# maksimt/rri_nmf

Hardware: AMD Instinct MI355X
Metric: RRI sweeps/sec and achieved HBM GB/s on dense X (n x d, rank k) (higher is better)
Workload: dtype f64

## Files before the change

### include/rri_hip.h

```cpp
#ifndef RRI_HIP_H
#define RRI_HIP_H

#include <stdint.h>
#include <stddef.h>

#ifdef __cplusplus
extern "C" {
#endif

#define RRI_ABI_VERSION 1
#define RRI_GRAM_SLICES 8
#define RRI_MAX_K 1024
#define RRI_MAX_TOPN 64
#define RRI_MAX_COOC_WORDS 32

typedef struct rri_ctx rri_ctx;
typedef struct rri_comm rri_comm;
#define RRI_COMM_ID_BYTES 128

typedef int32_t rri_status;
enum {
    RRI_OK = 0,
    RRI_PAUSED = 1,
    RRI_ERR_INVALID = -1,
// ... 83 lines not shown
rri_status rri_rank_entries(rri_ctx* ctx, const int64_t* rows, int64_t count,
                            const int64_t* tgt_indptr, const int32_t* tgt_indices,
                            const int64_t* excl_indptr, const int32_t* excl_indices,
                            double clip_lo, double clip_hi,
                            int32_t* rank_out, double* val_out, int32_t* eligible_out);
rri_status rri_cooccurrence_counts(rri_ctx* ctx, const int64_t* indptr, const int32_t* indices,
                                   int64_t n_rows, int64_t n_cols,
                                   const int32_t* words, int32_t n_groups, int32_t group_size,
                                   int64_t* df_out, int64_t* codf_out);
rri_status rri_entries_loglik(rri_ctx* ctx, const int64_t* rows, int64_t count,
                              const int64_t* indptr, const int32_t* indices, const double* values,
                              double floor, double* ll_out, double* mass_out, int64_t* floored_out);
enum { RRI_I32 = 8, RRI_I64 = 9 };
#define RRI_CORPUS_INFO_FIELDS 10
typedef struct rri_corpus rri_corpus;
rri_status rri_corpus_create(rri_ctx* ctx, rri_corpus** out, int64_t n_rows, int64_t n_cols, int64_t nnz_stored,
                             const void* indptr, int32_t indptr_dtype, const void* indices, int32_t indices_dtype,
                             const void* values, int32_t values_dtype, int32_t on_device);
rri_status rri_corpus_destroy(rri_corpus* corpus);
rri_status rri_corpus_info(const rri_corpus* corpus, int64_t* out, int32_t n, double* ingest_ms);
rri_status rri_corpus_get(rri_ctx* ctx, const rri_corpus* corpus, int64_t* indptr_out, int32_t* indices_out, double* values_out);
rri_status rri_corpus_memory(int64_t* corpora, int64_t* bytes);
rri_status rri_corpus_cooccurrence_counts(rri_ctx* ctx, const rri_corpus* corpus, const int32_t* words, int32_t n_groups,
                                          int32_t group_size, int64_t* df_out, int64_t* codf_out);
rri_status rri_corpus_entries_loglik(rri_ctx* ctx, const rri_corpus* corpus, const int64_t* rows, double floor,
                                     double* ll_out, double* mass_out, int64_t* floored_out);
#define RRI_SPARSE_STORE_INFO_FIELDS 10
rri_status rri_upload_X_corpus(rri_ctx* ctx, const rri_corpus* corpus);
rri_status rri_sparse_store_get(rri_ctx* ctx, int32_t which, int64_t* info, int32_t n_info, int64_t* segptr, uint16_t* idx,
                                int32_t* perm, void* val, int32_t* work);
rri_status rri_snapshot(rri_ctx* ctx);
rri_status rri_rollback(rri_ctx* ctx);

rri_status rri_X_times(rri_ctx* ctx, const double* B, int32_t m, double* out);
rri_status rri_Xt_times(rri_ctx* ctx, const double* Q, int32_t m, double* out);
rri_status rri_range_finder(rri_ctx* ctx, const double* Q0, int32_t m, int32_t n_iter, int32_t transpose, double* Q_out,
                            double* B_out);
rri_status rri_sparse_range_finder(rri_ctx* ctx, const double* Q0, int32_t m, int32_t n_iter, int32_t transpose, double* Q_out,
                                   double* B_out);

rri_status rri_column_positive_counts(rri_ctx* ctx, double* df_out);
rri_status rri_scale_X(rri_ctx* ctx, const double* col_scale, int32_t normalize_rows);
rri_status rri_set_X_scales(rri_ctx* ctx, const double* row_scale, const double* col_scale);
rri_status rri_get_X_scales(rri_ctx* ctx, double* row_out, double* col_out);
rri_status rri_csr_column_positive_counts(rri_ctx* ctx, double* df_out);
rri_status rri_csr_scale_X(rri_ctx* ctx, const double* col_scale, int32_t normalize_rows, int64_t* zero_rows_out);
rri_status rri_set_uniform_rows(rri_ctx* ctx, const int32_t* rows, int64_t count, double value);
rri_status rri_get_uniform_rows(rri_ctx* ctx, int32_t* rows_out, int64_t capacity, int64_t* count_out, double* value_out);
rri_status rri_csr_scale_X_uniform(rri_ctx* ctx, const double* col_scale, int32_t normalize_rows, int64_t* uniform_rows_out);

rri_status rri_comm_unique_id(uint8_t* id_out );
rri_status rri_comm_create(rri_comm** out, const uint8_t* id, int32_t rank, int32_t world, int32_t device);
typedef int32_t (*rri_allreduce_fn)(void* user, double* buf, int64_t count);
typedef int32_t (*rri_allgather_fn)(void* user, const double* send, int64_t count, double* recv);
typedef int32_t (*rri_broadcast_fn)(void* user, double* buf, int64_t count, int32_t root);
rri_status rri_comm_create_host(rri_comm** out, int32_t rank, int32_t world, rri_allreduce_fn allreduce,
                                rri_allgather_fn allgather, rri_broadcast_fn broadcast, void* user);
rri_status rri_comm_destroy(rri_comm* comm);
rri_status rri_attach_comm(rri_ctx* ctx, rri_comm* comm, int64_t row_offset, int64_t n_global);
rri_status rri_comm_broadcast(rri_ctx* ctx, double* host, int64_t count, int32_t root);
rri_status rri_comm_allreduce_sum(rri_ctx* ctx, double* host, int64_t count);
rri_status rri_comm_stats(rri_ctx* ctx, int32_t* rank, int32_t* world, int64_t* allreduce_calls);

rri_status rri_reduce_buffer(rri_ctx* ctx, void** dev_ptr, int64_t* n_elems);
rri_status rri_bind_reduce_buffer(rri_ctx* ctx, void* dev_ptr, int64_t n_elems);
rri_status rri_topic_reduce_local(rri_ctx* ctx, int32_t t);
rri_status rri_reduce_read(rri_ctx* ctx, double* out, int64_t count);
rri_status rri_reduce_write(rri_ctx* ctx, const double* in, int64_t count);
rri_status rri_topic_finish(rri_ctx* ctx, int32_t t);
rri_status rri_topic_finish_w(rri_ctx* ctx, int32_t t);
rri_status rri_resid_row_argmax(rri_ctx* ctx, double* value, int64_t* local_row);
rri_status rri_reset_row(rri_ctx* ctx, int64_t local_row, double* row_out_host);
rri_status rri_poll(rri_ctx* ctx);
rri_status rri_objective_parts(rri_ctx* ctx, double out[3]);

rri_status rri_frozen_set(rri_ctx* ctx, const double* B, const double* A, const double* s, double c);
rri_status rri_frozen_get(rri_ctx* ctx, double* B_out, double* A_out, double* s_out, double* c_out, int64_t* rows_out);
rri_status rri_frozen_absorb(rri_ctx* ctx, double decay);

rri_status rri_timing_enable(rri_ctx* ctx, int32_t on);
rri_status rri_timing_read(rri_ctx* ctx, int32_t kernel_id, int64_t* launches, double* total_ms);
rri_status rri_synchronize(rri_ctx* ctx);
rri_status rri_onchip_info(rri_ctx* ctx, int32_t* eligible, int64_t* launches);
#define RRI_LAYOUT_FIELDS 28
rri_status rri_layout_info(rri_ctx* ctx, int64_t* out, int32_t n);
rri_status rri_onchip_fallbacks(rri_ctx* ctx, int64_t* fallbacks);
rri_status rri_device_memory(int64_t* buffers, int64_t* bytes);
rri_status rri_debug_xcc(rri_ctx* ctx, int32_t* out, int32_t count);
rri_status rri_sweep_until(rri_ctx* ctx, int32_t n_sweeps, double obj_prev, double stop_scale, double* obj_hist,
                           int32_t* sweeps_done);
rri_status rri_bench_rank1_update(rri_ctx* ctx, int32_t reps, double* avg_ms);
rri_status rri_bench_stream_copy(rri_ctx* ctx, int32_t reps, double* avg_ms);

#ifdef __cplusplus
}
#endif
#endif
```

### rri_nmf_amd/_capi.py

```python
import ctypes as C
import os

_PKG = os.path.dirname(os.path.abspath(__file__))
LIB_PATH = os.environ.get('RRI_HIP_LIB', os.path.join(_PKG, 'lib', 'librri_hip.so'))

RRI_GRAM_SLICES = 8
RRI_LAYOUT_FIELDS = 28
RRI_MAX_K = 1024
RRI_MAX_TOPN = 64
RRI_MAX_COOC_WORDS = 32
RRI_OK, RRI_PAUSED = 0, 1
RRI_ERR_INVALID, RRI_ERR_HIP, RRI_ERR_UNSUPPORTED = -1, -2, -3
RRI_ERR_UNBOUNDED, RRI_ERR_W_COL_ZERO, RRI_ERR_NOT_IMPLEMENTED, RRI_ERR_COMM = -4, -5, -6, -7
RRI_COMM_ID_BYTES = 128
RRI_F32, RRI_F64, RRI_F16 = 0, 1, 2
RRI_U8 = 4
RRI_I32, RRI_I64 = 8, 9
RRI_CORPUS_INFO_FIELDS = 10
RRI_SPARSE_STORE_INFO_FIELDS = 10
RRI_UNWEIGHTED, RRI_WEIGHTED_DENSE, RRI_WEIGHTED_SPARSE, RRI_UNWEIGHTED_RESIDUAL, RRI_UNWEIGHTED_SPARSE = 0, 1, 2, 3, 4
RESET_NONE, RESET_MAX_RESID_DOCUMENT, RESET_RANDOM = 0, 1, 2
EVENT_NONE, EVENT_RESET_T, EVENT_RESET_W = 0, 1, 2
ABI_VERSION = 1


class Params(C.Structure):
    _fields_ = [('fix_W', C.c_int32), ('fix_T', C.c_int32), ('project_T_each_iter', C.c_int32),
                ('has_t_row_sum', C.c_int32), ('has_w_row_sum', C.c_int32), ('reset_method', C.c_int32),
                ('resets_left', C.c_int32), ('reserved0', C.c_int32),
                ('t_row_sum', C.c_double), ('w_row_sum', C.c_double),
                ('reg_w_l1', C.c_double), ('reg_w_l2', C.c_double), ('reg_t_l1', C.c_double),
                ('reg_t_l2', C.c_double), ('eps_div', C.c_double)]


class Event(C.Structure):
    _fields_ = [('kind', C.c_int32), ('topic', C.c_int32), ('sweep', C.c_int32), ('resume_topic', C.c_int32)]


_P = C.c_void_p
_I32, _I64, _D = C.c_int32, C.c_int64, C.c_double
ALLREDUCE_FN = C.CFUNCTYPE(C.c_int32, C.c_void_p, C.POINTER(C.c_double), C.c_int64)
ALLGATHER_FN = C.CFUNCTYPE(C.c_int32, C.c_void_p, C.POINTER(C.c_double), C.c_int64, C.POINTER(C.c_double))
BROADCAST_FN = C.CFUNCTYPE(C.c_int32, C.c_void_p, C.POINTER(C.c_double), C.c_int64, C.c_int32)
PROTOTYPES = {
    'rri_abi_version': (C.c_uint32, []),
    'rri_create': (_I32, [C.POINTER(_P), _I64, _I64, _I32, _I32, _I32, _I32, _P]),
    'rri_destroy': (_I32, [_P]),
    'rri_last_error': (C.c_char_p, [_P]),
    'rri_upload_X': (_I32, [_P, _P, _I64, _I32]),
    'rri_upload_mask': (_I32, [_P, _P, _I64, _I32]),
    'rri_bind_X_device': (_I32, [_P, _P, _I64]),
    'rri_storage_error': (_I32, [_P, C.POINTER(_D)]),
    'rri_bind_mask_device': (_I32, [_P, _P, _I64]),
    'rri_upload_X_csr': (_I32, [_P, C.POINTER(_I64), C.POINTER(_I32), _P, _I64, _I32]),
    'rri_upload_mask_csr_pattern': (_I32, [_P, C.POINTER(_I64), C.POINTER(_I32), _P, _I64, _I32]),
    'rri_upload_observed_csr': (_I32, [_P, C.POINTER(_I64), C.POINTER(_I32), _P, _I64, _I32]),
    'rri_set_W': (_I32, [_P, _P, _I64, _I32]),
    'rri_set_T': (_I32, [_P, _P, _I64, _I32]),
    'rri_get_W': (_I32, [_P, _P, _I64, _I32]),
    'rri_get_T': (_I32, [_P, _P, _I64, _I32]),
    'rri_set_params': (_I32, [_P, C.POINTER(Params)]),
    'rri_sweep': (_I32, [_P, _I32, C.POINTER(_I32)]),
    'rri_resume': (_I32, [_P, C.POINTER(_I32)]),
    'rri_pending_event': (_I32, [_P, C.POINTER(Event)]),
    'rri_apply_reset_max_resid': (_I32, [_P, _I32, C.POINTER(_I64)]),
    'rri_apply_reset_vectors': (_I32, [_P, _I32, C.POINTER(_D), C.POINTER(_D)]),
    'rri_skip_reset': (_I32, [_P]),
    'rri_update_T_row': (_I32, [_P, _I32]),
    'rri_update_W_col': (_I32, [_P, _I32]),
    'rri_project_W_rows': (_I32, [_P, _D, C.POINTER(_D)]),
    'rri_objective': (_I32, [_P, C.POINTER(_D)]),
    'rri_argmax_rows': (_I32, [_P, C.POINTER(_I32)]),
    'rri_masked_rmse': (_I32, [_P, C.POINTER(_I64), C.POINTER(_D), _I64, _D, _D, C.POINTER(_D)]),
    'rri_topn_rows': (_I32, [_P, C.POINTER(_I64), _I64, _I32, C.POINTER(_I64), C.POINTER(_I32), _D, _D, C.POINTER(_I32),
                             C.POINTER(_D)]),
    'rri_rank_entries': (_I32, [_P, C.POINTER(_I64), _I64, C.POINTER(_I64), C.POINTER(_I32), C.POINTER(_I64), C.POINTER(_I32),
                                _D, _D, C.POINTER(_I32), C.POINTER(_D), C.POINTER(_I32)]),
    'rri_cooccurrence_counts': (_I32, [_P, C.POINTER(_I64), C.POINTER(_I32), _I64, _I64, C.POINTER(_I32), _I32, _I32,
                                       C.POINTER(_I64), C.POINTER(_I64)]),
    'rri_entries_loglik': (_I32, [_P, C.POINTER(_I64), _I64, C.POINTER(_I64), C.POINTER(_I32), C.POINTER(_D), _D,
                                  C.POINTER(_D), C.POINTER(_D), C.POINTER(_I64)]),
    'rri_corpus_create': (_I32, [_P, C.POINTER(_P), _I64, _I64, _I64, _P, _I32, _P, _I32, _P, _I32, _I32]),
    'rri_corpus_destroy': (_I32, [_P]),
    'rri_corpus_info': (_I32, [_P, C.POINTER(_I64), _I32, C.POINTER(_D)]),
    'rri_corpus_get': (_I32, [_P, _P, C.POINTER(_I64), C.POINTER(_I32), C.POINTER(_D)]),
    'rri_corpus_memory': (_I32, [C.POINTER(_I64), C.POINTER(_I64)]),
    'rri_corpus_cooccurrence_counts': (_I32, [_P, _P, C.POINTER(_I32), _I32, _I32, C.POINTER(_I64), C.POINTER(_I64)]),
    'rri_corpus_entries_loglik': (_I32, [_P, _P, C.POINTER(_I64), _D, C.POINTER(_D), C.POINTER(_D), C.POINTER(_I64)]),
    'rri_upload_X_corpus': (_I32, [_P, _P]),
    'rri_sparse_store_get': (_I32, [_P, _I32, C.POINTER(_I64), _I32, C.POINTER(_I64), C.POINTER(C.c_uint16), C.POINTER(_I32), _P,
# ... 135 lines not shown
```

### rri_nmf_amd/csrc/rri_hip.hip

```cpp
#include <hip/hip_runtime.h>
#include <dlfcn.h>
#include <rccl/rccl.h>

#include <algorithm>
#include <atomic>
#include <chrono>
#include <cmath>
#include <cstdarg>
#include <cstdio>
#include <mutex>
#include <set>
#include <cstdlib>
#include <cstring>
#include <string>
#include <type_traits>
#include <utility>
#include <vector>

#include "rri_hip.h"
#include "rri_layout.hpp"
#include "rri_pick.hpp"
#include "rri_kernels.hpp"
#include "rri_wrri_kernels.hpp"
#include "rri_sparse_kernels.hpp"
// ... 125 lines not shown
    bool xp_valid = false;
    bool xp_done = false;
    int xp_base = 0;
    i64 xp_flagged = 0, xp_tiles = 0;
    bool gfull_valid = false;
    double *Gfull = nullptr, *Wsweep0 = nullptr, *wsum_part = nullptr, *wsums = nullptr;
    double *Y2part = nullptr, *Z2part = nullptr, *dtv = nullptr, *dwv = nullptr, *wold = nullptr, *zeros = nullptr;
    i64 ldw = 0;
    int nsplit = 4;
    i64 red_elems = 0;
    bool sparse = false;
    i64 nnz = 0;
    int sp_max_row = 0, kp = 8;
    i64* sp_rowptr = nullptr;
    int* sp_col = nullptr;
    void *sp_x = nullptr, *sp_e = nullptr;
    double* sp_Tt = nullptr;
    struct SpCopy {
        int nblk = 1, bw = 1, lps = 64, nwork = 0;
        i64 nseg = 0, gdim = 0, count = 0;
        i64* segptr = nullptr;
        unsigned short* idx = nullptr;
        void* val = nullptr;
        int* perm = nullptr;
        SpWork* work = nullptr;
    } sp[2];
    bool sparse_x = false;
    SpWork* spx_work = nullptr;
    double spb_ms = 0.0;
    double* rowhat = nullptr;
    int* uni_rows = nullptr;
    i64 uni_n = 0;
    double uni_value = 0.0;
    double* uni_part = nullptr;
    enum { UNI_REQ_NONE = 0, UNI_REQ_COLLECT = 1, UNI_REQ_ZERO = 2 };
    int uni_req = UNI_REQ_NONE;
    const int* uni_req_rows = nullptr;
    i64 uni_req_n = 0;
    struct ObsReq {
        const i64* indptr;
        const int* indices;
        const double* values;
        i64 nnz;
    };
    const ObsReq* obs_req = nullptr;
    double* Cpart = nullptr;
    double* N2part = nullptr;
    unsigned* Mcols = nullptr;
    bool nw_mask = false;
    bool mcols_tried = false;
    double mask_density = 1.0;
    int cpart_rows = 0;
    bool wcorr = false;
    int wcorr_topic = 0, wcorr_nrb = 0;
    bool resid_fresh = false;
    bool dt_pending = false;
    bool explicit_resid = false;
    bool dw_pending = false;
    int dw_topic = 0;
    double* told = nullptr;
    double *Gpart = nullptr, *tpart = nullptr, *rowobj = nullptr, *rowpos = nullptr, *normpart = nullptr;
    double *dtmp = nullptr;
    double* objbuf = nullptr;
    i64* itmp = nullptr;
    i64* tpart_idx = nullptr;
    double *resetT = nullptr, *resetW = nullptr;
    DevState* st = nullptr;

    int npanels = 1, rpb = 1, nrb = 1, nwb = 1, ntb = 1;
    int gpart_n = 1;
    int ttpart_n = 0;
    int xy_rows = 0;
    int xy_stride = 1;
    int ntb32 = 1;
    int tpart_n = 1;

    rri_params prm{};
    bool have_params = false, have_X = false, have_W = false, have_T = false, have_M = false;


    bool carry_valid = false;
    int carry_topic = -1;
    double *Tearly = nullptr, *edot = nullptr, *Gearly = nullptr, *ent = nullptr, *wfp = nullptr;
    bool early_valid = false, carry_wfin = false;
    int early_topic = -1, wfin_topic = -1;
    long early_steps = 0;
    double* XYpart = nullptr;
    int xy_run = -1;
    bool xy_valid = false, x_sq_valid = false;
    bool obj_track_pending = false, obj_track_valid = false;
    double obj_track_value = 0.0;
    struct { bool active = false; double prev = 0.0, scale = 0.0; int n = 0; double* out = nullptr; } until;
    double *objhist = nullptr, *objdec = nullptr;
    double x_sq = 0.0;
    bool pending_wcheck = false;
    int pending_wcheck_topic = -1;

    bool paused = false;
    int run_total = 0;
    Cursor resume_at{0, 0, 0};
    bool resume_done = false;
    rri_event pending{RRI_EVENT_NONE, -1, 0, 0};

    bool resid_valid = false;
    bool skip_row_finish = false;
    int nwb256 = 1;

    rri_comm* comm = nullptr;
    i64 row_offset = 0, n_global = 0;
    double* ctail = nullptr;
    double* cand = nullptr;
    double *fzB = nullptr, *fzA = nullptr, *fzs = nullptr, *fztail = nullptr;
    double fz_c = 0.0;
    i64 fz_rows = 0;
    rri_status comm_status = RRI_OK;

    int n_cu = 0;
    double *mkZ = nullptr, *mkG = nullptr, *mkP = nullptr, *mkX = nullptr, *mkT = nullptr, *objE = nullptr;
    unsigned* mkbar = nullptr;
    long onchip_launches = 0;
    double *Wsafe = nullptr, *Tsafe = nullptr;
    bool onchip_in_flight = false;
    bool onchip_off = false;
    long long onchip_off_until = 0;
    bool onchip_saved_skip = false;
    long onchip_fallbacks = 0;

    int timing = 0;
    long timing_seq[9] = {0, 0, 0, 0, 0, 0, 0, 0, 0};
    std::vector<TimedLaunch> timed[9];
    std::vector<hipEvent_t> event_pool;

    std::string err;
};
static inline bool ro_pass_interleaved(const rri_ctx* c) { return rri::ro_pass_interleaved(c->ro_il, c->npanels, c->nrb); }

enum : unsigned {
    CH_X = 1u << 0,
    CH_M = 1u << 1,
    CH_W = 1u << 2,
    CH_T = 1u << 3,
    CH_SCRATCH = 1u << 4,
    CH_PENALTY = 1u << 5,
    CH_ENDED = 1u << 6,
    CH_T_ROW = 1u << 7,
    CH_W_COL = 1u << 8,
    CH_E_FOLLOWS = 1u << 9
};
static void changed(rri_ctx* c, unsigned what) {
    if (what) c->early_valid = false;
    if (what & (CH_X | CH_M | CH_W | CH_T | CH_SCRATCH | CH_ENDED | CH_T_ROW)) c->carry_wfin = false;
    if (what & (CH_X | CH_M | CH_W | CH_T | CH_SCRATCH | CH_ENDED)) {
        c->carry_valid = false;
        c->carry_topic = -1;
        c->resid_valid = false;
        c->xy_run = -1;
        c->xy_valid = false;
        c->obj_track_valid = false;
    }
    if (what & CH_T_ROW) { c->carry_valid = false; c->xy_valid = false; }
    if ((what & (CH_T_ROW | CH_W_COL)) && !(what & CH_E_FOLLOWS)) c->resid_valid = false;
    if (what & (CH_T_ROW | CH_W_COL | CH_PENALTY)) c->obj_track_valid = false;
    if (what & (CH_X | CH_T | CH_T_ROW)) { c->q_valid = false; c->gfull_valid = false; }
    if (what & CH_X) { c->x_sq_valid = false; c->xp_valid = false; c->xn_valid = false; c->xp_done = false; }
    if (what & CH_ENDED) c->pending_wcheck = false;
}
// ... 643 lines not shown
            if (e == hipSuccess) e = allow_lds<k_resid<SX, true, false>>(c, 160 * 1024);
            if (e == hipSuccess) e = allow_lds<k_resid<SX, false, true>>(c, 160 * 1024);
            if (e == hipSuccess) e = allow_lds<k_spx_pass<SX>>(c, SP_BLOCK_BYTES + 64);
        }
        return e;
    }
};

#define DISPATCH(c, expr)                       \
    do {                                        \
        if ((c)->dtype == RRI_F32) {            \
            typedef LaunchX<float> L;           \
            expr;                               \
        } else if ((c)->dtype == RRI_F64) {     \
            typedef LaunchX<double> L;          \
            expr;                               \
        } else {                                \
            f16_unreachable(c);                 \
        }                                       \
    } while (0)
#define DISPATCH_RO(c, expr)                    \
    do {                                        \
        if ((c)->dtype == RRI_F32) {            \
            typedef LaunchX<float> L;           \
            expr;                               \
        } else if ((c)->dtype == RRI_F64) {     \
            typedef LaunchX<double> L;          \
            expr;                               \
        } else if ((c)->dtype == RRI_F16) {     \
            typedef LaunchX<_Float16> L;        \
            expr;                               \
        } else {                                \
            typedef LaunchX<unsigned char> L;   \
            expr;                               \
        }                                       \
    } while (0)

struct LK {
    static int gpart_rows(const rri_ctx* c) { return c->gpart_n; }
    template <bool UPDATE>
    static void wcol_resid(rri_ctx* c, int t, int tn, int sweep) {
        TimedScope ts(c, 1);
        hipLaunchKernelGGL((k_wcol_resid<UPDATE>), dim3(c->nwb256), dim3(256), 0, c->stream, c->W, c->ldw, (int)c->n,
                           c->k, t, tn, (const double*)c->Ypart, c->npanels, (const double*)c->Ttpart, c->nsplit,
                           c->dwv, c->Gpart, sweep, kparams(c), c->st);
        c->gpart_n = c->nwb256;
    }
    static size_t wcol_shmem(const rri_ctx* c) { return (size_t)(2 * c->k + 2 + 256 + 64) * sizeof(double); }
    template <bool UPDATE, bool CARRY>
    static void wcol_src(rri_ctx* c, int t, int tn, int sweep, const double* ypart, int nslices) {
        TimedScope ts(c, 1);
        hipLaunchKernelGGL((k_wcol<UPDATE, CARRY>), dim3(c->nwb), dim3(256), wcol_shmem(c), c->stream, c->W, c->ldw,
                           (int)c->n, c->k, t, tn, ypart, nslices, (const double*)c->Ttpart, c->ttpart_n, c->Gpart,
                           c->XYpart + (i64)t * c->xy_stride, sweep, kparams(c), c->st);
        c->gpart_n = c->nwb;
        if (UPDATE) note_xy(c, t, c->nwb * WCOL_TILES);
    }
    static void note_xy(rri_ctx* c, int t, int rows) {
        if (t == 0) { c->xy_run = 1; c->xy_rows = rows; }
        else c->xy_run = (c->xy_run == t && c->xy_rows == rows) ? t + 1 : -1;
        c->xy_valid = c->xy_run == c->k;
    }
    template <bool UPDATE, bool CARRY>
    static void wcol(rri_ctx* c, int t, int tn, int sweep) {
        wcol_src<UPDATE, CARRY>(c, t, tn, sweep, (const double*)c->Ypart, c->npanels);
    }
    static void frozen_add(rri_ctx* c, int t, int tprev) {
        if (!c->fzB) return;
        hipLaunchKernelGGL(k_frozen_add, dim3((unsigned)((c->LD + 255) / 256)), dim3(256), 0, c->stream, c->red, c->LD, c->k, t,
                           tprev, (const double*)c->fzB, (const double*)c->fzA, (const double*)c->fzs);
    }
    static void reduce(rri_ctx* c) {
        const int nb = (int)((c->LD + 31) / 32) + GRAM_SLICES;
        hipLaunchKernelGGL(k_reduce, dim3(nb), dim3(1024), 0, c->stream, (const double*)c->Zpart, c->LD, c->nrb,
                           (const double*)c->Gpart, gpart_rows(c), c->k, c->red, (const DevState*)c->st);
    }
    static bool light(const rri_ctx* c) { return !(c->prm.project_T_each_iter && c->prm.has_t_row_sum); }
    static bool early_ok(const rri_ctx* c) {
        return c->sw.early_sums && c->Tearly && !c->weighted && !c->explicit_resid && !c->sparse && c->k > 1 && !c->prm.fix_T &&
               !c->prm.fix_W && !c->comm && light(c) && !(small(c) && !c->fzB && c->sw.trow_fused) && WCOL_TILES == 1 &&
               early_job_lds_doubles(c->k) <= 5 * (size_t)c->rpb + 4 * 8 * 72;
    }
    static EarlyJob early_job(const rri_ctx* c, int t, int tn) {
        return EarlyJob{(const double*)c->W, c->ldw, (int)c->n, c->k, t, tn, (const double*)c->Tearly, c->plan.nte, c->edot,
                        c->Gearly, c->ent, early_job_first(c->npanels * c->nrb, c->n_cu), c->plan.e_blocks, c->plan.e_tpb};
    }
    static void wfin(rri_ctx* c, int t, int tn, int sweep) {
        TimedScope ts(c, 1);
        const int nredb = (int)((c->LD + 31) / 32) + GRAM_SLICES;
        hipLaunchKernelGGL(k_wfin, dim3(nredb + c->plan.nwfin), dim3(1024), 0, c->stream, c->W, c->ldw, (int)c->n, c->k, t, tn,
                           (const double*)c->Ypart, c->npanels, (const double*)c->edot, (const double*)c->ent, c->Gpart,
                           c->wfp, c->nwb, c->XYpart + (i64)t * c->xy_stride, (const double*)c->Zpart, c->LD, c->nrb, (const double*)c->Gearly,
                           c->plan.e_blocks, c->red, nredb, sweep, kparams(c), c->st);
        c->gpart_n = c->nwb;
        c->early_steps += 1;
        note_xy(c, t, c->nwb * WCOL_TILES);
    }
    static void trow_early(rri_ctx* c, int t, int check_prev, int tprev, int sweep) {
        hipLaunchKernelGGL(k_trow_early, dim3(c->plan.nte), dim3(1024), 0, c->stream, c->T, c->LD, (int)c->d, c->k, t,
                           (const double*)c->red, c->LD, c->carry_wfin ? (const double*)c->wfp : (const double*)nullptr, c->nwb,
                           c->wfin_topic, c->xraw, c->tpart, c->Tearly, check_prev, tprev, sweep, kparams(c), c->st);
        c->tpart_n = c->ntb;
    }
    static void trow(rri_ctx* c, int t, int check_prev, int tprev, int sweep, bool force_final) {
        hipLaunchKernelGGL(k_trow_numer, dim3(c->ntb), dim3(128), 0, c->stream, c->T, c->LD, (int)c->d, c->k, t,
                           (const double*)c->red, c->LD, c->xraw, c->tpart, c->tpart_idx, check_prev, tprev, sweep,
                           kparams(c), c->st, resid_sched(c) ? 1 : 0, resid_sched(c) ? c->told : (double*)nullptr);
        c->tpart_n = c->ntb;
        trow_final_if_needed(c, t, sweep, force_final);
    }
    static bool small(const rri_ctx* c) { return rri::trow_small(gpart_rows(c), c->k, c->ntb32); }
    static void trow_small(rri_ctx* c, int t, int check_prev, int tprev, int sweep, bool force_final) {
        hipLaunchKernelGGL(k_trow_small, dim3(c->ntb32), dim3(1024), 0, c->stream, c->T, c->LD, (int)c->d, c->k, t,
                           (const double*)c->Zpart, c->nrb, (const double*)c->Gpart, gpart_rows(c), c->red, c->LD, c->xraw,
                           c->tpart, c->tpart_idx, check_prev, tprev, sweep, kparams(c), c->st, resid_sched(c) ? 1 : 0,
                           resid_sched(c) ? c->told : (double*)nullptr);
        c->tpart_n = c->ntb32;
        trow_final_if_needed(c, t, sweep, force_final);
    }
    static void trow_final_if_needed(rri_ctx* c, int t, int sweep, bool force_final) {
        if (!light(c) || force_final)
            hipLaunchKernelGGL(k_trow_final, dim3(1), dim3(1024), 0, c->stream, c->T, c->LD, (int)c->d, t, c->xraw,
                               (const double*)c->tpart, (const i64*)c->tpart_idx, c->tpart_n, sweep, kparams(c), c->st);
    }
    static void check_prev_only(rri_ctx* c, int tprev, int sweep, int pos) {
        hipLaunchKernelGGL(k_check_red, dim3(1), dim3(64), 0, c->stream, (const double*)c->red, c->LD, c->k, tprev,
                           sweep, pos, kparams(c), c->st);
    }
    static void tgram(rri_ctx* c, int t, int finish, int sweep) {
        c->ttpart_n = c->nsplit;
        hipLaunchKernelGGL(k_tgram, dim3(c->k, c->nsplit), dim3(256), 0, c->stream, (const double*)c->T, c->LD,
                           (int)c->d, c->k, t, c->Ttpart, (const double*)c->tpart, c->tpart_n, finish, sweep,
                           kparams(c), c->st);
    }
    static void scale_wcol(rri_ctx* c, int t) {
        hipLaunchKernelGGL(k_scale_wcol, dim3((unsigned)((c->n + 255) / 256)), dim3(256), 0, c->stream, c->W,
                           c->ldw, (int)c->n, t, (const DevState*)c->st);
    }
    static void check_wcol(rri_ctx* c, int tprev, int sweep, int pos) {
        hipLaunchKernelGGL(k_check_wcol, dim3(1), dim3(256), 0, c->stream, (const double*)c->Gpart, gpart_rows(c), c->k,
                           tprev, sweep, pos, kparams(c), c->st);
    }
    static void proj_rows(rri_ctx* c, double s, const double* svec) {
        hipLaunchKernelGGL(k_proj_rows, dim3((unsigned)((c->n + 255) / 256)), dim3(256), 0, c->stream, c->W, c->ldw, (int)c->n, c->k, s,
                           svec);
    }
    static void norms(rri_ctx* c, const double* A, i64 rows, i64 cols, i64 ld) {
        hipLaunchKernelGGL(k_norms, dim3(256), dim3(256), 0, c->stream, A, rows, cols, ld, c->normpart);
    }
    static void reset_commit(rri_ctx* c, int t) {
        const i64 m = std::max(c->n, c->d);
        hipLaunchKernelGGL(k_reset_commit, dim3((unsigned)((m + 255) / 256)), dim3(256), 0, c->stream, c->W, c->ldw,
                           c->T, c->LD, (int)c->n, (int)c->d, t, (const i64*)c->itmp, (const double*)c->xraw);
    }
    static void set_row_col(rri_ctx* c, int t, const double* trow, const double* wcolv) {
        const i64 m = std::max(c->n, c->d);
        hipLaunchKernelGGL(k_set_row_col, dim3((unsigned)((m + 255) / 256)), dim3(256), 0, c->stream, c->W, c->ldw,
                           c->T, c->LD, (int)c->n, (int)c->d, t, trow, wcolv);
    }
    static void argmax_rows(rri_ctx* c, int* out) {
        hipLaunchKernelGGL(k_argmax_rows, dim3((unsigned)((c->n + 255) / 256)), dim3(256), 0, c->stream,
                           (const double*)c->W, c->ldw, (int)c->n, c->k, out);
    }
    static void masked_sqerr(rri_ctx* c, const i64* ij, const double* vals, i64 count, double lo, double hi) {
        hipLaunchKernelGGL(k_masked_sqerr, dim3(256), dim3(256), 0, c->stream, (const double*)c->W, c->ldw,
                           (const double*)c->T, c->LD, c->k, ij, vals, count, lo, hi, c->normpart);
    }
    static hipError_t topn_rows(rri_ctx* c, const i64* rows, i64 count, int N, const i64* eptr, const int* eidx, double lo,
                                double hi, int* idx_out, double* val_out) {
        const hipError_t e = allow_lds<k_topn_rows>(c, 64 * 1024);
        if (e != hipSuccess) return e;
        TimedScope ts(c, 4);
        hipLaunchKernelGGL(k_topn_rows, dim3((unsigned)((count + TOPN_ROWS - 1) / TOPN_ROWS)), dim3(256), topn_lds_bytes(N),
                           c->stream, (const double*)c->W, c->ldw, (const double*)c->T, c->LD, (int)c->d, c->k, rows, count, N,
                           eptr, eidx, lo, hi, idx_out, val_out);
        return hipGetLastError();
    }
    static hipError_t rank_entries(rri_ctx* c, const i64* rows, const RankPiece* pieces, i64 npieces, const int* tidx,
                                   const i64* eptr, const int* eidx, double lo, double hi, int* rank_out, double* val_out,
                                   int* elig_out) {
        const hipError_t e = allow_lds<k_rank_entries>(c, (int)rank_lds_bytes());
        if (e != hipSuccess) return e;
        TimedScope ts(c, 5);
        hipLaunchKernelGGL(k_rank_entries, dim3((unsigned)((npieces + RANK_PIECES - 1) / RANK_PIECES)), dim3(256), rank_lds_bytes(),
// ... 216 lines not shown
    if (!c->comm && c->fzB && !c->prm.fix_T) {
        hipLaunchKernelGGL(k_colsum_tail, dim3(1), dim3(256), 0, c->stream, (const double*)c->Gpart, LK::gpart_rows(c),
                           c->k, c->fztail, (const DevState*)c->st);
        hipLaunchKernelGGL(k_frozen_add_tail, dim3(1), dim3(64), 0, c->stream, c->fztail, tprev, (const double*)c->fzs);
        hipLaunchKernelGGL(k_wcheck_tail, dim3(1), dim3(64), 0, c->stream, (const double*)c->fztail, tprev, sweep, pos,
                           kparams(c), c->st);
        return;
    }
    if (!c->comm) {
        if (c->weighted)
            hipLaunchKernelGGL(k_wcheck_wcol, dim3(1), dim3(256), 0, c->stream, (const double*)c->Gpart, c->nwb256, c->k,
                               tprev, sweep, pos, kparams(c), c->st, (double*)nullptr);
        else LK::check_wcol(c, tprev, sweep, pos);
        return;
    }
    if (c->weighted)
        hipLaunchKernelGGL(k_wcheck_wcol, dim3(1), dim3(256), 0, c->stream, (const double*)c->Gpart, c->nwb256, c->k,
                           tprev, sweep, pos, kparams(c), c->st, c->ctail);
    else
        hipLaunchKernelGGL(k_colsum_tail, dim3(1), dim3(256), 0, c->stream, (const double*)c->Gpart, LK::gpart_rows(c),
                           c->k, c->ctail, (const DevState*)c->st);
    comm_allreduce(c, c->ctail, 2);
    hipLaunchKernelGGL(k_wcheck_tail, dim3(1), dim3(64), 0, c->stream, (const double*)c->ctail, tprev, sweep, pos,
                       kparams(c), c->st);
}
void flush_wcheck(rri_ctx* c, int sweep, int pos) {
    if (c->pending_wcheck) wcheck_now(c, c->pending_wcheck_topic, sweep, pos);
    c->pending_wcheck = false;
}

void enqueue_prologue(rri_ctx* c, int t, int sweep) {
    flush_wcheck(c, sweep, t);
    LK::wcol<false, true>(c, t, t, sweep);
    DISPATCH_RO(c, (L::template pass<false, true>(c, t, t)));
    c->carry_valid = true;
    c->carry_wfin = false;
    c->carry_topic = t;
}

void enqueue_T_half(rri_ctx* c, int sweep, int t, bool standalone) {
    const bool early = LK::early_ok(c);
    if (c->carry_wfin && !early) c->carry_valid = false;
    if (!c->carry_valid || c->carry_topic != t) enqueue_prologue(c, t, sweep);
    {
        TimedScope ts(c, 2);
        const int chk = c->pending_wcheck ? 1 : 0;
        if (early) {
            if (!c->carry_wfin) LK::reduce(c);
            LK::frozen_add(c, t, chk ? c->pending_wcheck_topic : -1);
            LK::trow_early(c, t, chk, c->pending_wcheck_topic, sweep);
            LK::trow_final_if_needed(c, t, sweep, standalone);
        } else if (LK::small(c) && !c->comm && !c->fzB && c->sw.trow_fused) {
            LK::trow_small(c, t, chk, c->pending_wcheck_topic, sweep, standalone);
        } else {
            LK::reduce(c);
            comm_allreduce(c, c->red, c->LD + (i64)GRAM_SLICES * (c->k + 2));
            LK::frozen_add(c, t, chk ? c->pending_wcheck_topic : -1);
            LK::trow(c, t, chk, c->pending_wcheck_topic, sweep, standalone);
        }
        c->pending_wcheck = false;
        if (c->prm.fix_W && no_regs(c)) LK::scale_wcol(c, t);
    }
    changed(c, CH_T_ROW);
    if (early) { c->early_valid = true; c->early_topic = t; }
}

void enqueue_W_half(rri_ctx* c, int sweep, int t) {
    const int k = c->k;
    const bool carry_next = (k > 1) && !c->prm.fix_T;
    const int tn = (t + 1) % k;
    const int finish = (LK::light(c) && !c->prm.fix_T && !c->skip_row_finish) ? 1 : 0;
    c->skip_row_finish = false;
    TgramJob job{};
    if (c->prm.fix_T || c->sparse_x) {
        TimedScope ts(c, 2);
        LK::tgram(c, t, finish, sweep);
    } else {
        job = TgramJob{(const double*)c->T, c->LD, (int)c->d, c->k, t, c->Ttpart, (const double*)c->tpart, c->tpart_n,
                       c->nsplit, finish, sweep, kparams(c), c->st, c->k * c->nsplit};
        c->ttpart_n = c->nsplit;
    }
    const bool early = carry_next && LK::early_ok(c) && c->early_valid && c->early_topic == t;
    if (carry_next) {
        DISPATCH_RO(c, (L::template pass<true, true>(c, t, tn, job, early ? LK::early_job(c, t, tn) : EarlyJob{})));
        if (early) LK::wfin(c, t, tn, sweep);
        else LK::wcol<true, true>(c, t, tn, sweep);
        c->carry_valid = true;
        c->carry_topic = tn;
        c->pending_wcheck = true;
        c->pending_wcheck_topic = t;
    } else {
        if (c->prm.fix_T) {
            if (!c->q_valid) {
                DISPATCH_RO(c, L::xtt(c));
                c->q_valid = true;
            }
            LK::wcol_src<true, false>(c, t, tn, sweep, c->Qt + (i64)t * c->ldw, 1);
        } else {
            DISPATCH_RO(c, (L::template pass<true, false>(c, t, tn, job)));
            LK::wcol<true, false>(c, t, tn, sweep);
        }
        const StepPos next = next_step(sweep, t, k);
        wcheck_now(c, t, next.sweep, next.pos);
        c->carry_valid = false;
    }
    changed(c, CH_W_COL);
    c->carry_wfin = early;
    c->wfin_topic = t;
}

void r_refresh(rri_ctx* c) {
    DISPATCH(c, L::resid(c, false, true, nullptr, nullptr));
    resid_rebuilt(c);
}

void enqueue_rT_half(rri_ctx* c, int sweep, int t, bool standalone) {
    if (!c->resid_valid) r_refresh(c);
    if (!c->carry_valid || c->carry_topic != t) {
        flush_wcheck(c, sweep, t);
        if (c->dw_pending) r_refresh(c);
        LK::wcol_resid<false>(c, t, t, sweep);
        DISPATCH(c, L::rpass_colsums(c, t));
        c->carry_valid = true;
        c->carry_topic = t;
    }
    {
        TimedScope ts(c, 2);
        const int chk = c->pending_wcheck ? 1 : 0;
        if (LK::small(c) && !c->comm) {
            LK::trow_small(c, t, chk, c->pending_wcheck_topic, sweep, standalone);
        } else {
            LK::reduce(c);
            comm_allreduce(c, c->red, c->LD + (i64)GRAM_SLICES * (c->k + 2));
            LK::trow(c, t, chk, c->pending_wcheck_topic, sweep, standalone);
        }
        c->pending_wcheck = false;
    }
    changed(c, CH_T_ROW | CH_E_FOLLOWS);
    c->resid_fresh = false;
    c->dt_pending = true;
}

void enqueue_rW_half(rri_ctx* c, int sweep, int t) {
    const int k = c->k;
    const int tn = (t + 1) % k;
    if (!c->resid_valid) r_refresh(c);
    const int finish = (LK::light(c) && !c->skip_row_finish) ? 1 : 0;
    c->skip_row_finish = false;
    const TgramJob job{(const double*)c->T, c->LD, (int)c->d, c->k, t, c->Ttpart, (const double*)c->tpart, c->tpart_n,
                       c->nsplit, finish, sweep, kparams(c), c->st, c->k * c->nsplit};
    c->ttpart_n = c->nsplit;
    const double* trow = c->T + (i64)t * c->LD;
    DISPATCH(c, {
        typename L::Upd u;
        u.a = c->dw_pending ? c->dwv : c->zeros;
        u.b = c->T + (i64)(c->dw_pending ? c->dw_topic : t) * c->LD;
        u.a2 = c->W + (i64)t * c->ldw;
        u.b2 = trow;
        u.b2sub = c->dt_pending ? c->told : trow;
        L::rank_update(c, c->E, c->LD, u, trow, c->W + (i64)tn * c->ldw, job);
    });
    LK::wcol_resid<true>(c, t, tn, sweep);
    changed(c, CH_W_COL | CH_E_FOLLOWS);
    c->dw_pending = true;
    c->dw_topic = t;
    c->dt_pending = false;
    c->resid_fresh = false;
// ... 552 lines not shown
    return true;
}

void enqueue_from(rri_ctx* c, Cursor cur) {
    if (cur.sweep < c->run_total && onchip_ok(c) && enqueue_onchip(c, cur)) return;
    if (c->until.active && cur.sweep < c->run_total) c->run_total = cur.sweep + 1;
    enqueue_range(c, cur, c->run_total);
    flush_wcheck(c, c->run_total, 0);
}

rri_status read_state(rri_ctx* c, DevState* out) {
    HIPCHK(c, hipMemcpyAsync(out, c->st, sizeof(DevState), hipMemcpyDeviceToHost, c->stream));
    HIPCHK(c, hipStreamSynchronize(c->stream));
    if (c->comm_status != RRI_OK) {
        const rri_status r = c->comm_status;
        c->comm_status = RRI_OK;
        changed(c, CH_ENDED);
        return r;
    }
    return RRI_OK;
}

rri_status status_from_halt(rri_ctx* c, const DevState& s, int32_t* sweeps_done) {
    if (s.halt == 0) {
        c->paused = false;
        if (sweeps_done) *sweeps_done = c->run_total;
        return RRI_OK;
    }
    changed(c, CH_ENDED);
    if (s.halt == HALT_EVENT_STOP) {
        c->paused = false;
        if (sweeps_done) *sweeps_done = s.halt_sweep;
        return RRI_OK;
    }
    if (s.halt > 0) {
        if (c->until.active) c->run_total = std::min(c->run_total, (s.halt == HALT_EVENT_RESET_W && s.halt_pos == 0) ? s.halt_sweep : s.halt_sweep + 1);
        c->paused = true;
        c->pending.kind = s.halt == HALT_EVENT_RESET_T ? RRI_EVENT_RESET_T : RRI_EVENT_RESET_W;
        c->pending.topic = s.halt_topic;
        c->pending.sweep = s.halt_sweep;
        c->pending.resume_topic = s.halt_pos;
        if (s.halt == HALT_EVENT_RESET_T) c->resume_at = Cursor{s.halt_sweep, s.halt_topic, 1};
        else c->resume_at = Cursor{s.halt_sweep, s.halt_pos, 0};
        if (sweeps_done) *sweeps_done = s.halt_sweep;
        return RRI_PAUSED;
    }
    c->paused = false;
    if (sweeps_done) *sweeps_done = s.halt_sweep;
    switch (s.halt) {
        case HALT_ERR_UNBOUNDED:
            return fail(c, RRI_ERR_UNBOUNDED, "Minimum objective is unbounded (topic %d)", s.halt_topic);
        case HALT_ERR_W_COL_ZERO:
            return fail(c, RRI_ERR_W_COL_ZERO, "W[:, t] sums to 0 (topic %d)", s.halt_topic);
        case HALT_ERR_NOT_IMPLEMENTED:
            return fail(c, RRI_ERR_NOT_IMPLEMENTED, "s=%g is not yet implemented", c->prm.t_row_sum);
        case HALT_ERR_GRID_SYNC:
            return fail(c, RRI_ERR_HIP, "the persistent sweep's workgroups could not synchronise (not all resident); RRI_ONCHIP=0 selects the launch-per-phase schedule");
        default:
            return fail(c, RRI_ERR_INVALID, "unknown device status %d", s.halt);
    }
}

rri_status clear_halt(rri_ctx* c) {
    HIPCHK(c, hipMemsetAsync(c->st, 0, 32, c->stream));
    return RRI_OK;
}

rri_switches read_switches() {
    rri_switches sw;
    if (const char* e = getenv("RRI_ONCHIP")) sw.onchip = atoi(e) != 0;
    if (const char* e = getenv("RRI_ONCHIP_OBJ")) sw.onchip_obj = atoi(e) != 0;
    if (const char* e = getenv("RRI_WSWEEP")) sw.wsweep = atoi(e) != 0;
    if (const char* e = getenv("RRI_TROW_SMALL")) sw.trow_fused = atoi(e) != 0;
    if (const char* e = getenv("RRI_OBJ_DIRECT")) sw.obj_direct = atoi(e) != 0;
    if (const char* e = getenv("RRI_WMCORR_COLS")) sw.wmcorr_cols = atoi(e) != 0;
    if (const char* e = getenv("RRI_WNW_MASK")) sw.wnw_mask = atoi(e) != 0;
    if (const char* e = getenv("RRI_PASS_ROT")) sw.pass_rot = atoi(e) & 7;
    if (const char* e = getenv("RRI_ROT_CAL")) sw.rot_cal = std::max(0, atoi(e));
    sw.rot_debug = getenv("RRI_ROT_DEBUG") != nullptr;
    if (const char* e = getenv("RRI_MASK_BITS")) sw.mask_bits = atoi(e) != 0;
    if (const char* e = getenv("RRI_PASS_CACHE_MB")) sw.pass_cache_mb = std::max(0.0, atof(e));
    if (const char* e = getenv("RRI_X_PACK")) sw.x_pack = atoi(e) == 2 ? 2 : atoi(e) != 0;
    if (const char* e = getenv("RRI_EARLY_SUMS")) sw.early_sums = atoi(e) != 0;
    if (const char* e = getenv("RRI_PASS_PK_GEOM")) {
        char* end = nullptr;
        sw.pk_rows = (int)std::min<long>(std::max<long>(0, strtol(e, &end, 10)), 1 << 20);
        sw.pk_il = (end && *end == 'i') ? 1 : (end && *end == 'c') ? 0 : -1;
    }
    return sw;
}

const char* sparse_data_refusal(const rri_ctx* c) {
    return c->sparse_x ? "an RRI_UNWEIGHTED_SPARSE handle keeps X as CSR: it takes its data through rri_upload_X_csr only "
                         "(no dense X, no device binding, no mask)"
                       : "a sparse-pattern handle takes its data through rri_upload_observed_csr";
}

#define REFUSE_RO(c, what)                                                                                              \
    if (ro_store((c)->dtype))                                                                                           \
        return fail((c), RRI_ERR_UNSUPPORTED, "%s is not available on an %s handle (%s stores a dense X that is only read)", what, \
                    dtype_name((c)->dtype), (c)->dtype == RRI_F16 ? "float16" : "uint8")

const char* const FROZEN_FIX_W_TEXT = "frozen statistics are set and fix_W is: the W[:,t] *= nt1 transfer of a T-row step would have to "
                                      "reach the frozen rows (clear the statistics, or let W move)";
bool frozen_fix_W(const rri_ctx* c) { return c->fzB && c->have_params && c->prm.fix_W; }
const char* frozen_refusal(const rri_ctx* c) {
    if (c->weighted == RRI_WEIGHTED_DENSE || c->weighted == RRI_WEIGHTED_SPARSE) return "a weighted handle sums its rows under a mask: frozen statistics are for unweighted handles";
    if (c->explicit_resid) return "the explicit-residual schedule keeps R = X - W T of its own rows: frozen statistics need the Gram form";
    if (ro_store(c->dtype)) return "frozen statistics are not available on an RRI_F16 or RRI_U8 handle";
    if (c->sparse_x && c->uni_n > 0) return "frozen statistics are not available on a CSR handle with uniform rows";
    if (c->comm) return "a communicator is attached: frozen statistics are for a handle on one device";
    return nullptr;
}
void frozen_release(rri_ctx* c) {
    dev_release(c, c->fzB); dev_release(c, c->fzA); dev_release(c, c->fzs); dev_release(c, c->fztail);
    c->fz_c = 0.0;
    c->fz_rows = 0;
}
hipError_t frozen_alloc(rri_ctx* c) {
    if (c->fzB) return hipSuccess;
    hipError_t e = dev_alloc(c, c->fzB, (size_t)c->k * c->LD * sizeof(double), true);
    if (e == hipSuccess) e = dev_alloc(c, c->fzA, (size_t)c->k * c->k * sizeof(double), true);
    if (e == hipSuccess) e = dev_alloc(c, c->fzs, (size_t)c->k * sizeof(double), true);
    if (e == hipSuccess) e = dev_alloc(c, c->fztail, 2 * sizeof(double), true);
    if (e != hipSuccess) frozen_release(c);
    return e;
}
void frozen_clear_topic_dev(rri_ctx* c, int t) {
    if (!c->fzB) return;
    const i64 m = std::max<i64>(c->LD, c->k);
    hipLaunchKernelGGL(k_frozen_clear, dim3((unsigned)((m + 255) / 256)), dim3(256), 0, c->stream, c->fzB, c->LD, c->fzA, c->k, c->fzs, t);
}

rri_status ready(rri_ctx* c) {
    if (!c->have_X || !c->have_W || !c->have_T || !c->have_params)
        return fail(c, RRI_ERR_INVALID, "X, W, T and params must be set before stepping");
    if (c->weighted && !c->have_M) return fail(c, RRI_ERR_INVALID, "weighted handle without a mask");
    return RRI_OK;
}

}

extern "C" {

uint32_t rri_abi_version(void) { return RRI_ABI_VERSION; }

const char* rri_last_error(const rri_ctx* ctx) { return ctx ? ctx->err.c_str() : g_create_error.c_str(); }

rri_status rri_create(rri_ctx** out, int64_t n, int64_t d, int32_t k, int32_t dtype, int32_t weighted,
                      int32_t device, void* stream) {
    if (!out) return RRI_ERR_INVALID;
    *out = nullptr;
    if (n < 1 || d < 1 || k < 1) return fail(nullptr, RRI_ERR_INVALID, "need n,d,k >= 1 (got %lld,%lld,%d)", n, d, k);
    if (dtype != RRI_F32 && dtype != RRI_F64 && dtype != RRI_F16 && dtype != RRI_U8)
        return fail(nullptr, RRI_ERR_INVALID, "dtype must be RRI_F32, RRI_F64, RRI_F16 or RRI_U8");
    if (n > 2000000000LL || d > 2000000000LL) return fail(nullptr, RRI_ERR_INVALID, "n, d must fit int32");
    if (k > RRI_MAX_K) return fail(nullptr, RRI_ERR_UNSUPPORTED, "k=%d is above the rank limit RRI_MAX_K = %d of the device path", k, RRI_MAX_K);
    int ndev = 0;
    if (hipGetDeviceCount(&ndev) != hipSuccess || ndev < 1)
        return fail(nullptr, RRI_ERR_HIP, "no HIP device available (librri_hip needs an MI355X)");
    if (device < 0 || device >= ndev) return fail(nullptr, RRI_ERR_INVALID, "device %d out of range [0,%d)", device, ndev);
    if (weighted < 0 || weighted > 4)
        return fail(nullptr, RRI_ERR_INVALID, "weighted must be RRI_UNWEIGHTED, RRI_WEIGHTED_DENSE, RRI_WEIGHTED_SPARSE, "
                                              "RRI_UNWEIGHTED_RESIDUAL or RRI_UNWEIGHTED_SPARSE");
    if (ro_store(dtype) && weighted != RRI_UNWEIGHTED) {
        static const struct { int dtype; const char *stores, *rewritten, *csr; } refusal[] = {
            {RRI_U8, "RRI_U8 stores read-only dense counts (RRI_UNWEIGHTED)", "keeps a stored residual, which counts 0..255 cannot hold",
             "keeps its values in a CSR store, which has no uint8 layout"},
            {RRI_F16, "RRI_F16 stores a read-only dense X (RRI_UNWEIGHTED)",
             "rewrites its stored residual at every topic step, which float16 would round every time",
             "keeps its values in a CSR store, which has no float16 layout"}};
        static const char* const flavour[] = {"", "RRI_WEIGHTED_DENSE", "RRI_WEIGHTED_SPARSE", "RRI_UNWEIGHTED_RESIDUAL", "RRI_UNWEIGHTED_SPARSE"};
        const bool rewritten = weighted == RRI_WEIGHTED_DENSE || weighted == RRI_UNWEIGHTED_RESIDUAL;
        for (const auto& r : refusal)
            if (r.dtype == dtype)
                return fail(nullptr, RRI_ERR_UNSUPPORTED, "%s; %s %s", r.stores, flavour[weighted], rewritten ? r.rewritten : r.csr);
    }
    rri_ctx* c = new rri_ctx();
    c->device = device;
#define CR(call)                                                                                   \
    do {                                                                                           \
        hipError_t e_ = (call);                                                                    \
        if (e_ != hipSuccess) {                                                                    \
            fail(nullptr, RRI_ERR_HIP, "%s failed: %s", #call, hipGetErrorString(e_));             \
            rri_destroy(c);                                                                        \
            return RRI_ERR_HIP;                                                                    \
        }                                                                                          \
    } while (0)
    CR(hipSetDevice(device));
    CR(hipDeviceGetAttribute(&c->n_cu, hipDeviceAttributeMultiprocessorCount, device));
    if (stream) c->stream = (hipStream_t)stream;
    else { CR(hipStreamCreateWithFlags(&c->stream, hipStreamNonBlocking)); c->own_stream = true; }

    c->sw = read_switches();
    const DensePlan p = c->plan = dense_plan(n, d, k, dtype, weighted, c->sw, c->n_cu);
    const bool explicit_resid = p.explicit_resid;
    weighted = p.weighted;
    c->explicit_resid = p.explicit_resid; c->sparse_x = p.sparse_x; c->sparse = p.sparse;
    c->n = n; c->d = d; c->k = k; c->dtype = dtype; c->weighted = weighted;
    c->kp = p.kp; c->es = dtype_size(dtype); c->VN = p.VN; c->PW = p.PW; c->LD = p.LD;
    c->npanels = p.npanels; c->rpb = p.rpb; c->nrb = p.nrb; c->ro_il = p.ro_il;
    for (int w = 0; w < 2 && p.sparse; ++w) {
        rri_ctx::SpCopy& cp = c->sp[w];
        cp.gdim = p.sp[w].gdim; cp.nseg = p.sp[w].nseg; cp.nblk = p.sp[w].nblk; cp.bw = p.sp[w].bw;
    }
    c->nwb = p.nwb; c->nwb256 = p.nwb256; c->ntb = p.ntb; c->ntb32 = p.ntb32; c->nsplit = p.nsplit;
    c->red_elems = p.red_elems; c->xy_stride = p.xy_stride; c->cpart_rows = p.cpart_rows;
    c->ldw = n;
    c->keep_q = pass_keep(c);
    c->tpart_n = c->ntb;
    c->gpart_n = c->nwb;
    c->ttpart_n = c->nsplit;

    const size_t f8 = sizeof(double);
    CR(dev_alloc(c, c->W, (size_t)k * c->ldw * f8));
    CR(dev_alloc(c, c->T, (size_t)k * c->LD * f8, true));
    CR(dev_alloc(c, c->Ypart, (size_t)c->npanels * n * f8, true));
    CR(dev_alloc(c, c->Zpart, (size_t)c->nrb * c->LD * f8, true));
    CR(dev_alloc(c, c->Gpart, (size_t)p.gpart_rows * (k + 2) * f8, true));
    CR(dev_alloc(c, c->XYpart, (size_t)k * c->xy_stride * f8, true));
    CR(dev_alloc(c, c->red, (size_t)c->red_elems * f8, true));
    CR(dev_alloc(c, c->xraw, (size_t)c->LD * f8, true));
    CR(dev_alloc(c, c->Ttpart, (size_t)p.ttpart_rows * k * f8, true));
    CR(dev_alloc(c, c->Qt, (size_t)k * c->ldw * f8));
    const size_t ntp = (size_t)p.tpart_rows;
    CR(dev_alloc(c, c->tpart, ntp * f8, true));
    CR(dev_alloc(c, c->tpart_idx, ntp * sizeof(i64)));
    CR(dev_alloc(c, c->normpart, 256 * 3 * f8));
    CR(dev_alloc(c, c->objbuf, (size_t)(2 * k * k + k) * f8));
    CR(dev_alloc(c, c->dtmp, 16 * f8));
    CR(dev_alloc(c, c->itmp, 16 * sizeof(i64)));
    if (c->sw.early_sums && !weighted && !explicit_resid && !p.sparse && k > 1) {
        CR(dev_alloc(c, c->Tearly, (size_t)p.nte * k * f8, true));
        CR(dev_alloc(c, c->edot, (size_t)n * f8, true));
        CR(dev_alloc(c, c->Gearly, (size_t)p.e_blocks * (k + 2) * f8, true));
        CR(dev_alloc(c, c->ent, 8 * f8, true));
        CR(dev_alloc(c, c->wfp, (size_t)2 * c->nwb * f8, true));
    }
    const bool keeps_resid = explicit_resid || (weighted && !c->sparse);
    if (keeps_resid) CR(dev_alloc(c, c->E, (size_t)n * c->LD * c->es, c->LD != d));
    if (weighted) {
        CR(dev_alloc(c, c->Y2part, (size_t)c->npanels * n * f8, true));
        CR(dev_alloc(c, c->Z2part, (size_t)c->nrb * c->LD * f8, true));
        if (!c->sparse) {
            CR(dev_alloc(c, c->Cpart, (size_t)c->cpart_rows * c->LD * f8, true));
            CR(dev_alloc(c, c->N2part, (size_t)c->cpart_rows * c->LD * f8, true));
        }
        CR(dev_alloc(c, c->dtv, (size_t)c->LD * f8, true));
    }
    if (weighted || explicit_resid) CR(dev_alloc(c, c->dwv, (size_t)n * f8, explicit_resid));
    if (weighted) CR(dev_alloc(c, c->wold, (size_t)n * f8));
    if (explicit_resid) CR(dev_alloc(c, c->told, (size_t)c->LD * f8, true));
    if (weighted || explicit_resid) CR(dev_alloc(c, c->zeros, (size_t)std::max<i64>(c->LD, n) * f8, true));
    if (c->sparse) CR(dev_alloc(c, c->sp_Tt, (size_t)d * c->kp * f8, true));
    if (dtype == RRI_U8) {
        CR(dev_alloc(c, c->rscale, (size_t)n * f8));
        CR(dev_alloc(c, c->cscale, (size_t)c->LD * f8));
        hipLaunchKernelGGL(k_fill, dim3((unsigned)((n + 255) / 256)), dim3(256), 0, c->stream, c->rscale, (i64)n, 1.0);
        hipLaunchKernelGGL(k_fill, dim3((unsigned)((c->LD + 255) / 256)), dim3(256), 0, c->stream, c->cscale, c->LD, 1.0);
    }
    CR(dev_alloc(c, c->st, sizeof(DevState), true));
    if (dtype == RRI_F32) CR(LaunchX<float>::set_attrs(c));
    else if (dtype == RRI_F64) CR(LaunchX<double>::set_attrs(c));
    else if (dtype == RRI_F16) CR(LaunchX<_Float16>::set_attrs(c));
    else CR(LaunchX<unsigned char>::set_attrs(c));
    CR(hipStreamSynchronize(c->stream));
#undef CR
    *out = c;
    return RRI_OK;
}

rri_status rri_destroy(rri_ctx* c) {
    if (!c) return RRI_OK;
    (void)hipSetDevice(c->device);
    if (c->stream) (void)hipStreamSynchronize(c->stream);
    for (const auto& o : c->owned) {
        (void)hipFree(o.p);
        dev_count(-1, o.bytes);
    }
    for (int i = 0; i < 9; ++i)
        for (auto& tl : c->timed[i]) { (void)hipEventDestroy(tl.a); (void)hipEventDestroy(tl.b); }
    for (auto e : c->event_pool) (void)hipEventDestroy(e);
    if (c->own_stream && c->stream) (void)hipStreamDestroy(c->stream);
    delete c;
    return RRI_OK;
}

rri_status rri_upload_X(rri_ctx* c, const void* host, int64_t ld, int32_t host_dtype) {
    CHECK_CTX(c);
    if (c->sparse) return fail(c, RRI_ERR_UNSUPPORTED, "%s", sparse_data_refusal(c));
    if (rri_status s = check_host_matrix(c, host, ld, host_dtype, c->d, c->dtype)) return s;
    HIPCHK(c, hipSetDevice(c->device));
    if (!dev_owned(c, &c->X)) HIPCHK(c, dev_alloc(c, c->X, (size_t)c->n * c->LD * c->es, c->LD != c->d));
    c->ldx = c->LD;
    c->store_err[0] = c->store_err[1] = 0.0;
    rri_status s = to_device(c, host, ld, host_dtype, c->X, c->ldx, c->n, c->d, c->dtype);
    if (s == RRI_OK || ro_store(c->dtype)) { c->have_X = s == RRI_OK; changed(c, CH_X); }
    if (s == RRI_OK) s = reset_scales(c);
    return s;
}

rri_status rri_upload_mask(rri_ctx* c, const void* host, int64_t ld, int32_t host_dtype) {
    CHECK_CTX(c);
    REFUSE_RO(c, "a mask");
    if (c->sparse) return fail(c, RRI_ERR_UNSUPPORTED, "%s", sparse_data_refusal(c));
    if (!c->weighted) return fail(c, RRI_ERR_INVALID, "handle was not created with weighted=1");
    if (rri_status s = check_host_matrix(c, host, ld, host_dtype, c->d, c->dtype)) return s;
    HIPCHK(c, hipSetDevice(c->device));
    if (!dev_owned(c, &c->M)) HIPCHK(c, dev_alloc(c, c->M, (size_t)c->n * c->LD * c->es, c->LD != c->d));
    c->ldm = c->LD;
    rri_status s = to_device(c, host, ld, host_dtype, c->M, c->ldm, c->n, c->d, c->dtype);
    if (s == RRI_OK) {
        c->have_M = true;
        changed(c, CH_M);
        DISPATCH(c, s = L::pack_mask_if_binary(c));
        if (s != RRI_OK) return fail(c, s, "packing the mask failed");
        if (c->Mbits) dev_release(c, c->M);
    }
    return s;
// ... 2890 lines not shown
    if (m->nccl) {
        (void)hipSetDevice(m->device);
        (void)rccl_api().CommDestroy(m->nccl);
    }
    delete m;
    return RRI_OK;
}

rri_status rri_attach_comm(rri_ctx* c, rri_comm* comm, int64_t row_offset, int64_t n_global) {
    CHECK_CTX(c);
    if (comm && c->sparse_x) return fail(c, RRI_ERR_UNSUPPORTED, "an RRI_UNWEIGHTED_SPARSE handle is not row-sharded");
    if (comm && ro_store(c->dtype)) return fail(c, RRI_ERR_UNSUPPORTED, "an %s handle is not row-sharded (the combination has no test yet)", dtype_name(c->dtype));
    if (comm && c->fzB) return fail(c, RRI_ERR_UNSUPPORTED, "frozen statistics are set: clear them before a communicator is attached");
    if (!comm) {
        c->comm = nullptr;
        c->row_offset = 0;
        c->n_global = 0;
        changed(c, CH_SCRATCH);
        return RRI_OK;
    }
    if (row_offset < 0 || n_global < row_offset + c->n) return fail(c, RRI_ERR_INVALID, "row block [%lld, %lld) outside 0..%lld", (long long)row_offset, (long long)(row_offset + c->n), (long long)n_global);
    if (comm->nccl && comm->device != c->device) return fail(c, RRI_ERR_INVALID, "communicator lives on device %d, handle on %d", comm->device, c->device);
    HIPCHK(c, hipSetDevice(c->device));
    HIPCHK(c, dev_ensure(c, c->ctail, 8 * sizeof(double), true));
    dev_release(c, c->cand);
    HIPCHK(c, dev_alloc(c, c->cand, (size_t)2 * comm->world * sizeof(double)));
    c->comm = comm;
    c->row_offset = row_offset;
    c->n_global = n_global;
    c->comm_status = RRI_OK;
    changed(c, CH_SCRATCH);
    return RRI_OK;
}

rri_status rri_comm_broadcast(rri_ctx* c, double* host, int64_t count, int32_t root) {
    CHECK_CTX(c);
    if (!c->comm) return RRI_OK;
    if (!host || count < 1 || root < 0 || root >= c->comm->world) return fail(c, RRI_ERR_INVALID, "bad broadcast arguments");
    HIPCHK(c, hipSetDevice(c->device));
    DevTmp buf;
    HIPCHK(c, buf.alloc((size_t)count * sizeof(double)));
    HIPCHK(c, hipMemcpyAsync(buf.p, host, (size_t)count * 8, hipMemcpyHostToDevice, c->stream));
    comm_broadcast(c, (double*)buf.p, count, root);
    HIPCHK(c, hipMemcpyAsync(host, buf.p, (size_t)count * 8, hipMemcpyDeviceToHost, c->stream));
    HIPCHK(c, hipStreamSynchronize(c->stream));
    if (c->comm_status != RRI_OK) { const rri_status r = c->comm_status; c->comm_status = RRI_OK; return r; }
    return RRI_OK;
}

rri_status rri_comm_allreduce_sum(rri_ctx* c, double* host, int64_t count) {
    CHECK_CTX(c);
    if (!host || count < 1) return fail(c, RRI_ERR_INVALID, "bad all-reduce arguments");
    HIPCHK(c, hipSetDevice(c->device));
    if (count <= 8 || !c->comm) return comm_allreduce_host(c, host, count);
    DevTmp buf;
    HIPCHK(c, buf.alloc((size_t)count * sizeof(double)));
    HIPCHK(c, hipMemcpyAsync(buf.p, host, (size_t)count * 8, hipMemcpyHostToDevice, c->stream));
    comm_allreduce(c, (double*)buf.p, count);
    HIPCHK(c, hipMemcpyAsync(host, buf.p, (size_t)count * 8, hipMemcpyDeviceToHost, c->stream));
    HIPCHK(c, hipStreamSynchronize(c->stream));
    if (c->comm_status != RRI_OK) { const rri_status r = c->comm_status; c->comm_status = RRI_OK; return r; }
    return RRI_OK;
}

rri_status rri_comm_stats(rri_ctx* c, int32_t* rank, int32_t* world, int64_t* allreduce_calls) {
    CHECK_CTX(c);
    if (rank) *rank = c->comm ? c->comm->rank : 0;
    if (world) *world = c->comm ? c->comm->world : 1;
    if (allreduce_calls) *allreduce_calls = c->comm ? c->comm->n_allreduce : 0;
    return RRI_OK;
}

rri_status rri_onchip_info(rri_ctx* c, int32_t* eligible, int64_t* launches) {
    CHECK_CTX(c);
    if (eligible) *eligible = (c->have_X && c->have_params && onchip_ok(c)) ? 1 : 0;
    if (launches) *launches = c->onchip_launches;
    return RRI_OK;
}

rri_status rri_layout_info(rri_ctx* c, int64_t* out, int32_t n) {
    CHECK_CTX(c);
    if (!out || n < 1) return fail(c, RRI_ERR_INVALID, "rri_layout_info needs room for at least one value");
    const bool dense_w = c->weighted == RRI_WEIGHTED_DENSE;
    const int64_t v[RRI_LAYOUT_FIELDS] = {
        c->sparse ? c->sp[0].nblk : 0, c->sparse ? c->sp[0].bw : 0, c->sparse ? c->sp[0].lps : 0, c->sparse ? c->sp[0].nwork : 0,
        c->sparse ? c->sp[1].nblk : 0, c->sparse ? c->sp[1].bw : 0, c->sparse ? c->sp[1].lps : 0, c->sparse ? c->sp[1].nwork : 0,
        c->rpb, c->nrb, c->npanels,
        c->Mbits ? 1 : 0, c->Mcols ? 1 : 0,
        c->mcols_tried && c->Mbits ? (int64_t)(c->mask_density * 1.0e9 + 0.5) : -1,
        dense_w && wtrow_small(c) ? 1 : 0,
        dense_w && c->nw_mask ? 1 : 0,
        !c->sparse && ro_pass_interleaved(c) ? 1 : 0,
        c->wcorr_nrb, c->n_cu,
        c->xp_valid ? 1 : 0, c->xp_valid ? c->xp_base : 0, c->xp_flagged, c->xp_tiles,
        c->xp_valid ? (c->xn_valid ? 26 : 28) : 0, c->xn_valid ? (int64_t)((uint64_t)c->xn_books.hi << 32 | c->xn_books.lo) : 0,
        c->xn_exceptions,
        LK::early_ok(c) ? 1 : 0, c->early_steps};
    for (int i = 0; i < n && i < RRI_LAYOUT_FIELDS; ++i) out[i] = v[i];
    return RRI_OK;
}

rri_status rri_device_memory(int64_t* buffers, int64_t* bytes) {
    if (buffers) *buffers = g_dev_buffers.load();
    if (bytes) *bytes = g_dev_bytes.load();
    return RRI_OK;
}

rri_status rri_debug_xcc(rri_ctx* c, int32_t* out, int32_t count) {
    CHECK_CTX(c);
    if (!out || count < 1 || count > 4096) return fail(c, RRI_ERR_INVALID, "bad count");
    HIPCHK(c, hipSetDevice(c->device));
    DevTmp dv;
    HIPCHK(c, dv.alloc((size_t)count * sizeof(int)));
    hipLaunchKernelGGL(k_xcc_probe, dim3((unsigned)count), dim3(64), 0, c->stream, (int*)dv.p);
    HIPCHK(c, hipMemcpyAsync(out, dv.p, (size_t)count * sizeof(int), hipMemcpyDeviceToHost, c->stream));
    HIPCHK(c, hipStreamSynchronize(c->stream));
    return RRI_OK;
}

rri_status rri_onchip_fallbacks(rri_ctx* c, int64_t* fallbacks) {
    CHECK_CTX(c);
    if (fallbacks) *fallbacks = c->onchip_fallbacks;
    return RRI_OK;
}

rri_status rri_timing_enable(rri_ctx* c, int32_t on) {
    CHECK_CTX(c);
    c->timing = on < 0 ? 0 : on;
    for (int i = 0; i < 9; ++i) c->timing_seq[i] = 0;
    return RRI_OK;
}

rri_status rri_timing_read(rri_ctx* c, int32_t id, int64_t* launches, double* total_ms) {
    CHECK_CTX(c);
    if (id < 0 || id > 8) return fail(c, RRI_ERR_INVALID, "kernel_id out of range");
    HIPCHK(c, hipSetDevice(c->device));
    HIPCHK(c, hipStreamSynchronize(c->stream));
    double tot = 0.0;
    for (auto& tl : c->timed[id]) {
        float ms = 0.f;
        HIPCHK(c, hipEventElapsedTime(&ms, tl.a, tl.b));
        tot += ms;
        c->event_pool.push_back(tl.a);
        c->event_pool.push_back(tl.b);
    }
    if (launches) *launches = (int64_t)c->timed[id].size();
    if (total_ms) *total_ms = tot;
    c->timed[id].clear();
    return RRI_OK;
}

rri_status rri_synchronize(rri_ctx* c) {
    CHECK_CTX(c);
    HIPCHK(c, hipSetDevice(c->device));
    HIPCHK(c, hipStreamSynchronize(c->stream));
    return RRI_OK;
}

static size_t x_span_bytes(const rri_ctx* c) { return ((size_t)(c->n - 1) * c->ldx + c->LD) * c->es; }

rri_status rri_bench_stream_copy(rri_ctx* c, int32_t reps, double* avg_ms) {
    CHECK_CTX(c);
    REFUSE_RO(c, "the stream-copy yardstick");
    if (!c->have_X || reps < 1 || c->sparse) return fail(c, RRI_ERR_INVALID, "a dense X must be set and reps >= 1");
    HIPCHK(c, hipSetDevice(c->device));
    const size_t bytes = x_span_bytes(c);
    DevTmp dst;
    EventPair ev;
    HIPCHK(c, dst.alloc(bytes));
    HIPCHK(c, ev.create());
    const i64 nvec = (i64)(bytes / 16);
    hipLaunchKernelGGL(k_stream_copy, dim3(256 * 8), dim3(256), 0, c->stream, (const float4*)c->X, (float4*)dst.p, nvec);
    (void)hipEventRecord(ev.a, c->stream);
    for (int r = 0; r < reps; ++r)
        hipLaunchKernelGGL(k_stream_copy, dim3(256 * 8), dim3(256), 0, c->stream, (const float4*)c->X, (float4*)dst.p, nvec);
    (void)hipEventRecord(ev.b, c->stream);
    hipError_t e = hipStreamSynchronize(c->stream);
    float ms = 0.f;
    (void)hipEventElapsedTime(&ms, ev.a, ev.b);
    if (e != hipSuccess) return fail(c, RRI_ERR_HIP, "stream copy failed: %s", hipGetErrorString(e));
// ... 162 lines not shown
```

### rri_nmf_amd/csrc/rri_kernels.hpp

```cpp
#pragma once
#include <type_traits>

#include "rri_device.hpp"
#include "rri_halt.hpp"
#include "rri_hip.h"
#include "rri_layout.hpp"
#include "rri_xnarrow.hpp"
#include "rri_xpack.hpp"

namespace rri {

typedef float f32x4 __attribute__((ext_vector_type(4)));
typedef double f64x2 __attribute__((ext_vector_type(2)));
typedef unsigned u32x4 __attribute__((ext_vector_type(4)));
typedef unsigned u32x2 __attribute__((ext_vector_type(2)));
typedef unsigned __attribute__((may_alias)) u32_any;

template <typename SX> struct XVec;
template <> struct XVec<float> {
    typedef f32x4 type;
    static constexpr int N = 4;
    static __device__ __forceinline__ void unpack(const f32x4& v, double (&o)[4]) {
        o[0] = (double)v[0]; o[1] = (double)v[1]; o[2] = (double)v[2]; o[3] = (double)v[3];
    }
    static __device__ __forceinline__ f32x4 pack(const double (&o)[4]) {
        return f32x4{(float)o[0], (float)o[1], (float)o[2], (float)o[3]};
    }
    static __device__ __forceinline__ f32x4 zero() { return f32x4{0.f, 0.f, 0.f, 0.f}; }
};
template <> struct XVec<double> {
    typedef f64x2 type;
    static constexpr int N = 2;
    static __device__ __forceinline__ void unpack(const f64x2& v, double (&o)[2]) { o[0] = v[0]; o[1] = v[1]; }
    static __device__ __forceinline__ f64x2 pack(const double (&o)[2]) { return f64x2{o[0], o[1]}; }
    static __device__ __forceinline__ f64x2 zero() { return f64x2{0.0, 0.0}; }
};
typedef _Float16 f16x8 __attribute__((ext_vector_type(8)));
typedef _Float16 f16x4 __attribute__((ext_vector_type(4)));
template <> struct XVec<_Float16> {
    typedef f16x8 type;
    static constexpr int N = 8;
    static __device__ __forceinline__ void unpack(const f16x8& v, double (&o)[8]) {
#pragma unroll
        for (int e = 0; e < 8; ++e) o[e] = (double)(float)v[e];
    }
    static __device__ __forceinline__ f16x8 pack(const double (&o)[8]) {
        f16x8 r;
#pragma unroll
        for (int e = 0; e < 8; ++e) r[e] = (_Float16)(float)o[e];
        return r;
    }
    static __device__ __forceinline__ f16x8 zero() {
        return f16x8{(_Float16)0.f, (_Float16)0.f, (_Float16)0.f, (_Float16)0.f, (_Float16)0.f, (_Float16)0.f, (_Float16)0.f, (_Float16)0.f};
    }
};

typedef unsigned char u8x8 __attribute__((ext_vector_type(8)));
template <> struct XVec<unsigned char> {
    typedef u8x8 type;
    static constexpr int N = 8;
    static __device__ __forceinline__ void unpack(const u8x8& v, double (&o)[8]) {
#pragma unroll
        for (int e = 0; e < 8; ++e) o[e] = (double)(float)v[e];
    }
    static __device__ __forceinline__ u8x8 pack(const double (&o)[8]) {
        u8x8 r;
#pragma unroll
        for (int e = 0; e < 8; ++e) r[e] = (unsigned char)o[e];
        return r;
    }
    static __device__ __forceinline__ u8x8 zero() { return u8x8{0, 0, 0, 0, 0, 0, 0, 0}; }
};
struct XScale {
    const double* row;
    const double* col;
};
template <typename SX> constexpr bool XSCALED = std::is_same<SX, unsigned char>::value;
template <typename SX>
__device__ __forceinline__ double x_elem(const SX* __restrict__ X, i64 ldx, i64 i, i64 j, const XScale& xs) {
    if constexpr (XSCALED<SX>) return ((double)(float)X[i * ldx + j] * xs.col[j]) * xs.row[i];
    else return (double)X[i * ldx + j];
}

template <bool NT, typename V>
__device__ __forceinline__ V stream_load(const V* p) {
    if constexpr (NT) return __builtin_nontemporal_load(p);
    else return *p;
}

template <bool NT, typename V>
__device__ __forceinline__ void stream_store(V* p, const V& v) {
    if constexpr (NT) __builtin_nontemporal_store(v, p);
    else *p = v;
}

struct TgramJob {
    const double* T; i64 ldt; int d, k, t;
    double* Ttpart; const double* tpart; int ntb, nsplit, finish, sweep;
    KParams p; DevState* st;
    int nblocks;
};
__device__ __forceinline__ void tgram_block(const double* __restrict__ T, i64 ldt, int d, int k, int t, int l, int split,
                                            int ns, double* __restrict__ Ttpart, const double* __restrict__ tpart,
                                            int nblk, int finish, int sweep, const KParams& p, DevState* st,
                                            double* scratch) {
    const int chunk = (d + ns - 1) / ns;
    const int j0 = split * chunk, j1 = min(d, j0 + chunk);
    double acc = 0.0;
    for (int j = j0 + threadIdx.x; j < j1; j += 256) acc = fma(T[(i64)l * ldt + j], T[(i64)t * ldt + j], acc);
    acc = block_sum(acc, scratch);
    if (threadIdx.x == 0) Ttpart[split * k + l] = acc;
    if (finish && l == 0 && split == 0) {
        double ps = 0.0;
        ps = ordered_sum<4>(tpart, 1, threadIdx.x, nblk, 256);
        ps = block_sum(ps, scratch);
        if (threadIdx.x == 0) {
            const int mode = st->tmode;
            st->nt1 = (mode == 0) ? ps : 1.0;
            st->sumT = ps;
            if (trow_resets(ps, p)) halt_set(st, HALT_EVENT_RESET_T, t, sweep, t);
        }
    }
}

struct EarlyJob {
    const double* Wt; i64 ldw; int n, k, t, tn;
    const double* Tearly; int nte;
    double *dot, *Gpart, *nt;
    int first, nblocks, tpb;
};
template <int CH>
__device__ __forceinline__ void early_block(const EarlyJob& e, int b, double* sm) {
    const int tid = threadIdx.x, lane = tid & 63, wave = tid >> 6, k = e.k, t = e.t;
    double* tts = sm;
    double* gsh = tts + k;
    double* dsh = gsh + k + 2;
    for (int l = tid; l < k + 2; l += 256) gsh[l] = 0.0;
    for (int l = tid; l < k; l += 256) tts[l] = ordered_sum<8>(e.Tearly + l, k, 0, e.nte, 1);
    __syncthreads();
    if (b == 0 && tid == 0) e.nt[0] = tts[t];
    __syncthreads();
    if (tid == 0) tts[t] = 0.0;
    __syncthreads();
    const int ntiles = (e.n + 63) / 64;
    const int tile1 = min(ntiles, (b + 1) * e.tpb);
    for (int tile = b * e.tpb; tile < tile1; ++tile) {
        const i64 i = (i64)tile * 64 + lane;
        const bool valid = i < e.n;
        const double wn = valid ? e.Wt[(i64)e.tn * e.ldw + i] : 0.0;
        double dotv = 0.0;
        for (int l0 = wave; l0 < k; l0 += 4 * CH) {
            double wl[CH];
#pragma unroll
            for (int q = 0; q < CH; ++q) {
                const int l = l0 + 4 * q;
                wl[q] = (l < k && valid && l != t) ? e.Wt[(i64)l * e.ldw + i] : 0.0;
            }
#pragma unroll
            for (int q = 0; q < CH; ++q) {
                const int l = l0 + 4 * q;
                if (l < k) {
                    dotv = fma(wl[q], tts[l], dotv);
                    if (l != t) {
                        const double g = wave_sum<double>(wn * wl[q]);
                        if (lane == 0) gsh[l] += g;
                    }
                }
            }
        }
        dsh[wave * 64 + lane] = dotv;
        __syncthreads();
        if (wave == 0) {
            if (valid) e.dot[i] = (dsh[lane] + dsh[64 + lane]) + (dsh[128 + lane] + dsh[192 + lane]);
            const double nwp = wave_sum<double>(wn * wn);
            if (lane == 0) gsh[k] += nwp;
        }
        __syncthreads();
    }
    double* gp = e.Gpart + (i64)b * (k + 2);
    for (int l = tid; l < k + 2; l += 256) gp[l] = gsh[l];
}

#define RRI_PASS_ROW_SUMS \
            double yp = 0.0;                                                                                      \
        _Pragma("unroll")                                                                                         \
            for (int e = 0; e < VN; ++e) {                                                                        \
                if (DO_Y) yp = fma(xe[e], tv[e], yp);                                                             \
                if (DO_Z) zacc[e] = fma(wv, xe[e], zacc[e]);                                                      \
            }                                                                                                     \
            if constexpr (DO_Y && RS) wave_rowsum8_park(tile, u, lane, yp);                                       \
            else if (DO_Y) {                                                                                      \
                 \
                const double tot = wave_sum_lane63<double>(yp);                                                   \
                if (lane == 63) ysh[wave * rpb + l0 + u] = tot;                                                   \
            }
#define RRI_PASS_CHUNK_SUMS \
        if constexpr (DO_Y && RS) {                                                                               \
            const double tot = wave_rowsum8_finish(tile, lane);                                                   \
            if ((lane & 7) == 0) ysh[wave * rpb + l0 + (lane >> 3)] = tot;                                        \
        }

#define RRI_PASS_ROWS(LNT) \
    for (int l0 = 0; l0 < rpb; l0 += U) {                                                                         \
        const int r = grow(l0);                                        \
        if (r >= n) break;                                               \
        V x[U];                                                                                                   \
        _Pragma("unroll")                                                                                         \
        for (int u = 0; u < U; ++u) {                                                                             \
            const int rr = r + u;                                                                                 \
            x[u] = XV::zero();                                                                                    \
            if (rr < n && ok) x[u] = stream_load<LNT>(reinterpret_cast<const V*>(X + (i64)rr * ldx + col));       \
        }                                                                                                         \
        _Pragma("unroll")                                                                                         \
        for (int u = 0; u < U; ++u) {                                                                             \
            const int rr = r + u;                                                                                 \
            double wv = 0.0, na = 0.0, na2 = 0.0;                                                                 \
            if (DO_Z && rr < n) wv = wsh[l0 + u];                                                                 \
            if (UPD > 0 && rr < n) na = -ash[l0 + u];                                                             \
            if (UPD > 1 && rr < n) na2 = -ash2[l0 + u];                                                           \
            double xe[VN];                                                                                        \
            XV::unpack(x[u], xe);                                                                                 \
            if constexpr (UPD > 0) {                                                                              \
// ... 29 lines not shown
        _Pragma("unroll")                                                                                         \
        for (int u = 0; u < U; ++u) {                                                                             \
            const int rr = r + u;                                                                                 \
            double wv = 0.0;                                                                                      \
            if (DO_Z && rr < n) wv = wsh[l0 + u];                                                                 \
            unsigned xb[4];                                                                                       \
            xpack::decode_row(xw, u, base4, xb);                                                                  \
            double xe[VN];                                                                                        \
        _Pragma("unroll")                                                                                         \
            for (int e = 0; e < VN; ++e) xe[e] = (double)__uint_as_float(xb[e]);                                  \
            RRI_PASS_ROW_SUMS                                                                                     \
        }                                                                                                         \
        RRI_PASS_CHUNK_SUMS                                                                                       \
    }

#define RRI_PASS_ROWS_PN(LNT) \
    {                                                                                                             \
        unsigned char* const mapb = reinterpret_cast<unsigned char*>(tile);                                       \
        u32_any* const mapw = reinterpret_cast<u32_any*>(tile);                                                   \
        constexpr unsigned MAP_ROW = 72 * sizeof(double);                                                         \
        const unsigned wpanel = (unsigned)(pg * 4 + wave), wpanels = (unsigned)npg * 4u;                          \
        unsigned e0 = 0u, e1 = 0u;                                                                                \
        if (grow(0) < n) {                                                                                        \
            const unsigned long long ri0 = xnarrow::record_index((unsigned)grow(0) >> 3, wpanel, wpanels);        \
            e0 = xdir[ri0]; e1 = xdir[ri0 + 1];                                                                   \
        }                                                                                                         \
        for (int l0 = 0; l0 < rpb; l0 += U) {                                                                     \
            const int r = grow(l0);                                                                               \
            if (r >= n) break;                                                                                    \
            const unsigned long long ri = xnarrow::record_index((unsigned)r >> 3, wpanel, wpanels);               \
            const unsigned char* recb = XP + ri * xnarrow::RECORD_BYTES;                                          \
            unsigned en = 0u;                                                                                     \
            if (e0 + (unsigned)lane < e1) en = xexc[e0 + (unsigned)lane];                                         \
            unsigned n0 = 0u, n1 = 0u;                                                                            \
            if (l0 + U < rpb && grow(l0 + U) < n) {                                                               \
                const unsigned long long rin = xnarrow::record_index((unsigned)grow(l0 + U) >> 3, wpanel, wpanels); \
                n0 = xdir[rin]; n1 = xdir[rin + 1];                                                               \
            }                                                                                                     \
            unsigned xw[xnarrow::LANE_DWORDS];                                                                    \
        _Pragma("unroll")                                                                                         \
            for (int i = 0; i < (int)xnarrow::WIDE_SLOTS; ++i) {                                                  \
                u32x4 v = u32x4{0u, 0u, 0u, 0u};                                                                  \
                if (ok) v = stream_load<LNT>(reinterpret_cast<const u32x4*>(recb) + i * (int)xnarrow::LANES + lane); \
                xw[4 * i] = v[0]; xw[4 * i + 1] = v[1]; xw[4 * i + 2] = v[2]; xw[4 * i + 3] = v[3];               \
            }                                                                                                     \
            {                                                                                                     \
                u32x2 v = u32x2{0u, 0u};                                                                          \
                if (ok) v = stream_load<LNT>(reinterpret_cast<const u32x2*>(recb + xnarrow::dword_offset(24u, 0u)) + lane); \
                xw[24] = v[0]; xw[25] = v[1];                                                                     \
            }                                                                                                     \
        _Pragma("unroll")                                                                                         \
            for (int u = 0; u < U; ++u) mapw[u * (int)(MAP_ROW / 4u) + lane] = 0u;                                \
            if (e0 + (unsigned)lane < e1)                                                                         \
                mapb[xnarrow::map_offset(en & 2047u, MAP_ROW)] = (unsigned char)xnarrow::rare_entry(xbooks, en >> xnarrow::POS_BITS); \
            for (unsigned b = e0 + 64u; b < e1; b += 64u) {       \
                const unsigned j = b + (unsigned)lane;                                                            \
                if (j < e1) {                                                                                     \
                    const unsigned en2 = xexc[j];                                                                 \
                    mapb[xnarrow::map_offset(en2 & 2047u, MAP_ROW)] = (unsigned char)xnarrow::rare_entry(xbooks, en2 >> xnarrow::POS_BITS); \
                }                                                                                                 \
            }                                                                                                     \
            asm volatile("s_waitcnt lgkmcnt(0)" ::: "memory");                                                    \
            __builtin_amdgcn_wave_barrier();                                                                      \
        _Pragma("unroll")                                                                                         \
            for (int u = 0; u < U; ++u) {                                                                         \
                const int rr = r + u;                                                                             \
                double wv = 0.0;                                                                                  \
                if (DO_Z && rr < n) wv = wsh[l0 + u];                                                             \
                const unsigned mapped = mapw[u * (int)(MAP_ROW / 4u) + lane];                                     \
                unsigned xb[4];                                                                                   \
                xnarrow::decode_row(xw, u, mapped, xbooks.lo, xbooks.hi, xb);                                     \
                double xe[VN];                                                                                    \
        _Pragma("unroll")                                                                                         \
                for (int e = 0; e < VN; ++e) xe[e] = (double)__uint_as_float(xb[e]);                              \
                RRI_PASS_ROW_SUMS                                                                                 \
            }                                                                                                     \
            RRI_PASS_CHUNK_SUMS                                                                                   \
            if constexpr (!(DO_Y && RS)) __builtin_amdgcn_wave_barrier();                                         \
            e0 = n0; e1 = n1;                                                                                     \
        }                                                                                                         \
    }

template <typename SX, bool DO_Y, bool DO_Z, int UPD, int U, bool NT, bool RS, int PK = 0, bool EJ = false>
__global__ __launch_bounds__(256) void k_pass(typename std::conditional<(UPD > 0), SX, const SX>::type* __restrict__ X,
                                              i64 ldx, int n, int ncols,
                                              const double* __restrict__ trow, const double* __restrict__ wcol,
                                              double* __restrict__ Ypart, double* __restrict__ Zpart, i64 ldz,
                                              int rpb, int npg, const double* __restrict__ avec,
                                              const double* __restrict__ bvec, const double* __restrict__ avec2,
                                              const double* __restrict__ bvec2, const double* __restrict__ bsub2,
                                              const DevState* __restrict__ st, const TgramJob job, int nrb_il_rot,
                                              int keep_q, const unsigned char* __restrict__ XP = nullptr,
                                              const unsigned char* __restrict__ xflags = nullptr, int xbase = 0,
                                              const double* __restrict__ rscale = nullptr,
                                              const double* __restrict__ cscale = nullptr,
                                              const unsigned* __restrict__ xdir = nullptr,
                                              const unsigned short* __restrict__ xexc = nullptr,
                                              const xnarrow::Books xbooks = xnarrow::Books{},
                                              const EarlyJob ejob = EarlyJob{}) {
    static_assert(!XSCALED<SX> || UPD == 0, "counts with scales are only read");
    static_assert(!PK || (std::is_same<SX, float>::value && UPD == 0 && U == 8), "the packed copy is of a read-only fp32 X");
    static_assert(!EJ || (DO_Y && DO_Z && UPD == 0), "the early-sums job rides in the fused read-only pass");
    typedef XVec<SX> XV;
    typedef typename XV::type V;
    constexpr int VN = XV::N;
    constexpr int PW = 64 * VN;
    if (st->halt) return;
    if ((int)blockIdx.x < job.nblocks) {
        __shared__ double jscratch[40];
        tgram_block(job.T, job.ldt, job.d, job.k, job.t, (int)blockIdx.x % job.k, (int)blockIdx.x / job.k, job.nsplit,
                    job.Ttpart, job.tpart, job.ntb, job.finish, job.sweep, job.p, job.st, jscratch);
        return;
    }
    const int nrb_il = nrb_il_rot & 0x07ffffff;
    const int rot = (int)((unsigned)nrb_il_rot >> 27);
    extern __shared__ __attribute__((aligned(16))) unsigned char smem[];
    int bid = (int)blockIdx.x - job.nblocks;
    int njobs = job.nblocks;
    if constexpr (EJ) {
        if (bid >= ejob.first && bid < ejob.first + ejob.nblocks) {
            early_block<(sizeof(SX) == 8 ? 4 : 8)>(ejob, bid - ejob.first, reinterpret_cast<double*>(smem));
            return;
        }
        if (bid >= ejob.first) bid -= ejob.nblocks;
        njobs += ejob.nblocks;
    }
    if (rot != 0 && (bid | 7) < (int)gridDim.x - njobs) bid = (bid & ~7) | ((bid + rot) & 7);
    double* ysh = reinterpret_cast<double*>(smem);
    double* wsh = ysh + 4 * rpb;
    double* ash = wsh + rpb;
    double* ash2 = ash + rpb;
    static_assert(!RS || U == 8, "the LDS row-sum path reduces 8 rows at a time");
    const int lane = threadIdx.x & 63;
    const int wave = __builtin_amdgcn_readfirstlane(threadIdx.x >> 6);
    double* tile = wsh + (1 + UPD) * rpb + wave * (8 * 72);
    const int pg = bid % npg;
    const int rb = bid / npg;
    auto grow = [&](int li) -> int {
        return nrb_il > 0 ? ((li / U) * nrb_il + rb) * U + (li % U) : rb * rpb + li;
    };
    const int col = (pg * 4 + wave) * PW + lane * VN;
    int xflag = 0;
    if constexpr (PK) {
        for (int l0 = (int)threadIdx.x * U; l0 < rpb; l0 += 256 * U) {
            const int g = grow(l0);
            if (g < n) xflag |= xflags[(i64)(g >> 3) * npg + pg];
        }
    }
    if (DO_Z || UPD > 0) {
        for (int i = threadIdx.x; i < rpb; i += 256) {
            const int g = grow(i);
            if constexpr (XSCALED<SX>) { if (DO_Z) wsh[i] = g < n ? wcol[g] * rscale[g] : 0.0; }
            else if (DO_Z) wsh[i] = g < n ? wcol[g] : 0.0;
            if (UPD > 0) ash[i] = g < n ? avec[g] : 0.0;
            if (UPD > 1) ash2[i] = g < n ? avec2[g] : 0.0;
        }
        if constexpr (PK) xflag = __syncthreads_or(xflag);
        else __syncthreads();
    } else if constexpr (PK) xflag = __syncthreads_or(xflag);
    const unsigned base4 = (unsigned)xbase * 0x01010101u;
    const bool ok = col < ncols;
    const bool wave_has_cols = (pg * 4 + wave) * PW < ncols;
    double tv[VN], zacc[VN], bv[VN], bv2[VN];
#pragma unroll
    for (int e = 0; e < VN; ++e) {
        zacc[e] = 0.0;
        if constexpr (XSCALED<SX>) tv[e] = (DO_Y && ok) ? trow[col + e] * cscale[col + e] : 0.0;
        else tv[e] = (DO_Y && ok) ? trow[col + e] : 0.0;
        bv[e] = (UPD > 0 && ok) ? bvec[col + e] : 0.0;
        bv2[e] = (UPD > 1 && ok) ? bvec2[col + e] - bsub2[col + e] : 0.0;
    }
    if (wave_has_cols) {
        if constexpr (PK && NT) {
            const unsigned nrb = ((unsigned)gridDim.x - (unsigned)njobs) / (unsigned)npg;
            const bool kept = ((unsigned)(rb + 1) * (unsigned)keep_q) / nrb != ((unsigned)rb * (unsigned)keep_q) / nrb;
            if constexpr (PK == 2) {
                if (xflag) { RRI_PASS_ROWS(true) }
                else if (kept) { RRI_PASS_ROWS_PN(false) }
                else { RRI_PASS_ROWS_PN(true) }
            } else {
                if (xflag) { RRI_PASS_ROWS(true) }
                else if (kept) { RRI_PASS_ROWS_PK(false) }
                else { RRI_PASS_ROWS_PK(true) }
            }
        } else if constexpr (PK == 2) {
            if (xflag) { RRI_PASS_ROWS(false) }
            else { RRI_PASS_ROWS_PN(false) }
        } else if constexpr (PK) {
            if (xflag) { RRI_PASS_ROWS(false) }
            else { RRI_PASS_ROWS_PK(false) }
        } else if constexpr (NT && UPD == 0) {
            const unsigned nrb = ((unsigned)gridDim.x - (unsigned)njobs) / (unsigned)npg;
// ... 515 lines not shown
    if (st->halt) return;
    __shared__ double scratch[40];
    const i64 i = (i64)blockIdx.x * 256 + threadIdx.x;
    double cden = 1.0, nt = 0.0;
    int mode = 0;
    if (UPDATE) {
        nt = ordered_sum<8>(Ttpart + t, k, 0, nsplit, 1);
        cden = nt + p.reg_w_l2;
        mode = wcol_denominator_mode(cden, p);
        if (mode < 0) {
            if (blockIdx.x == 0 && threadIdx.x == 0) halt_set(st, mode, t, sweep, t);
            return;
        }
    }
    double wnew = 0.0, dwi = 0.0, wn = 0.0;
    if (i < n) {
        if (UPDATE) {
            const double y = ordered_sum<8>(Ypart + i, n, 0, npanels, 1);
            const double w0 = Wt[(i64)t * ldw + i];
            const double numer = fma(w0, nt, y) - p.reg_w_l1;
            if (mode == 0) wnew = fmax(numer, 0.0) / (cden + p.eps);
            else wnew = (-numer + cden < 0.0) ? p.w_row_sum : 0.0;
            Wt[(i64)t * ldw + i] = wnew;
            dwi = wnew - w0;
            dw[i] = dwi;
        }
        wn = (UPDATE && tn == t) ? wnew : Wt[(i64)tn * ldw + i];
    }
    const double g = block_sum(wn * dwi, scratch);
    const double nwp = block_sum(wn * wn, scratch);
    const double sw = block_sum(wnew, scratch);
    double* gp = Gpart + (i64)blockIdx.x * (k + 2);
    for (int l = threadIdx.x; l < k + 2; l += 256) gp[l] = (l == t && UPDATE) ? g : (l == k ? nwp : (l == k + 1 ? sw : 0.0));
}

__device__ __forceinline__ void reduce_block(int bx, int nb, const double* __restrict__ Zpart, i64 ldz, int nrb,
                                             const double* __restrict__ Gpart, int nwb, int k, double* __restrict__ red,
                                             double* sh) {
    const int tid = threadIdx.x;
    const int ngram = Gpart ? GRAM_SLICES : 0;
    const int nzb = nb - ngram;
    if (bx < nzb) {
        const int c = tid & 31, g = tid >> 5;
        const i64 j = (i64)bx * 32 + c;
        double a = 0.0;
        if (j < ldz) a = ordered_sum<8>(Zpart + j, ldz, g, nrb, 32);
        sh[g * 33 + c] = a;
        __syncthreads();
        if (tid < 32 && j < ldz) {
            double s = 0.0;
            for (int q = 0; q < 32; ++q) s += sh[q * 33 + tid];
            red[j] = s;
        }
    } else {
        const int gs = bx - nzb;
        const int per = (nwb + GRAM_SLICES - 1) / GRAM_SLICES;
        const int b0 = gs * per, b1 = min(nwb, b0 + per);
        const int lane = tid & 63, wave = tid >> 6;
        for (int l0 = 0; l0 < k + 2; l0 += 64) {
            const int l = l0 + lane;
            double a = 0.0;
            if (l < k + 2) a = ordered_sum<8>(Gpart + l, k + 2, b0 + wave, b1, 16);
            __syncthreads();
            sh[wave * 64 + lane] = a;
            __syncthreads();
            if (wave == 0 && l < k + 2) {
                double s = 0.0;
                for (int q = 0; q < 16; ++q) s += sh[q * 64 + lane];
                red[ldz + (i64)gs * (k + 2) + l] = s;
            }
        }
    }
}
__global__ __launch_bounds__(1024) void k_reduce(const double* __restrict__ Zpart, i64 ldz, int nrb,
                                                 const double* __restrict__ Gpart, int nwb, int k,
                                                 double* __restrict__ red, const DevState* __restrict__ st) {
    if (st->halt) return;
    __shared__ double sh[32 * 33];
    reduce_block((int)blockIdx.x, (int)gridDim.x, Zpart, ldz, nrb, Gpart, nwb, k, red, sh);
}

__global__ __launch_bounds__(1024) void k_wfin(double* __restrict__ Wt, i64 ldw, int n, int k, int t, int tn,
                                               const double* __restrict__ Ypart, int npanels,
                                               const double* __restrict__ dot, const double* __restrict__ nt,
                                               double* __restrict__ Gtile, double* __restrict__ wfp, int ntiles,
                                               double* __restrict__ xyp, const double* __restrict__ Zpart, i64 ldz, int nrb,
                                               const double* __restrict__ Gearly, int ne, double* __restrict__ red,
                                               int nredb, int sweep, KParams p, DevState* st) {
    static_assert(WFIN_TILES == 16 && WCOL_TILES == 1, "a wave per tile, a row of Gtile and an entry of xyp per tile");
    if (st->halt) return;
    __shared__ double sh[32 * 33];
    if ((int)blockIdx.x < nredb) {
        reduce_block((int)blockIdx.x, nredb, Zpart, ldz, nrb, Gearly, ne, k, red, sh);
        return;
    }
    const int b = (int)blockIdx.x - nredb;
    const int lane = threadIdx.x & 63, wave = threadIdx.x >> 6;
    const double cden = nt[0] + p.reg_w_l2;
    const int mode = wcol_denominator_mode(cden, p);
    if (mode < 0) {
        if (b == 0 && threadIdx.x == 0) halt_set(st, mode, t, sweep, t);
        return;
    }
    const i64 tile = (i64)b * 16 + wave;
    if (tile * 64 >= n) return;
    const i64 i = tile * 64 + lane;
    const bool valid = i < n;
    double wn = 0.0, y = 0.0, wnew = 0.0;
    if (valid) {
        wn = Wt[(i64)tn * ldw + i];
        const double dt = dot[i];
        y = ordered_sum<8>(Ypart + i, n, 0, npanels, 1);
        const double numer = (y - dt) - p.reg_w_l1;
        if (mode == 0) wnew = fmax(numer, 0.0) / (cden + p.eps);
        else wnew = (-numer + cden < 0.0) ? p.w_row_sum : 0.0;
        Wt[(i64)t * ldw + i] = wnew;
    }
    const double swp = wave_sum<double>(wnew);
    const double xy = wave_sum<double>(wnew * y);
    const double gt = wave_sum<double>(wn * wnew);
    if (lane == 0) {
        wfp[tile] = gt;
        wfp[ntiles + tile] = swp;
        Gtile[tile * (k + 2) + k + 1] = swp;
        xyp[tile] = xy;
    }
}

__device__ __forceinline__ double red_gram(const double* __restrict__ red, i64 ldz, int k, int l) {
    double s = 0.0;
#pragma unroll
    for (int g = 0; g < GRAM_SLICES; ++g) s += red[ldz + (i64)g * (k + 2) + l];
    return s;
}

__global__ __launch_bounds__(128) void k_trow_numer(double* __restrict__ T, i64 ldt, int d, int k, int t,
                                                    const double* __restrict__ red, i64 ldz,
                                                    double* __restrict__ xraw, double* __restrict__ tpart,
                                                    i64* __restrict__ tpart_idx, int check_prev, int tprev,
                                                    int sweep, KParams p, DevState* st, int resid_form,
                                                    double* __restrict__ told) {
    if (st->halt) return;
    const int tid = threadIdx.x;
    __shared__ double scratch[40];
    __shared__ double gsh[RRI_MAX_K];
    const double nw = red_gram(red, ldz, k, k);
    if (check_prev) {
        const int code = wcol_code(red_gram(red, ldz, k, k + 1), p);
        if (code != 0) {
            if (blockIdx.x == 0 && tid == 0) halt_set(st, code, tprev, sweep, t);
            return;
        }
    }
    const double c = nw + p.reg_t_l2;
    const bool project = p.project_T && p.has_trs;
    const int mode = trow_denominator_mode(c, p);
    if (mode < 0) {
        if (blockIdx.x == 0 && tid == 0) halt_set(st, mode, t, sweep, t);
        return;
    }
    for (int l = tid; l < k; l += 128) gsh[l] = (l == t) ? (resid_form ? -nw : 0.0) : red_gram(red, ldz, k, l);
    __syncthreads();
    const i64 j = (i64)blockIdx.x * 128 + tid;
    double x = 0.0, mx = -1.0e300;
    if (j < d) {
        if (told) told[j] = T[(i64)t * ldt + j];
        double a0 = 0.0, a1 = 0.0, a2 = 0.0, a3 = 0.0;
        for (int l0 = 0; l0 < k; l0 += 16) {
            double tv[16];
#pragma unroll
            for (int q = 0; q < 16; ++q) tv[q] = (l0 + q < k) ? T[(i64)(l0 + q) * ldt + j] : 0.0;
#pragma unroll
            for (int q = 0; q < 16; q += 4) {
                if (l0 + q < k) a0 = fma(gsh[l0 + q], tv[q], a0);
                if (l0 + q + 1 < k) a1 = fma(gsh[l0 + q + 1], tv[q + 1], a1);
                if (l0 + q + 2 < k) a2 = fma(gsh[l0 + q + 2], tv[q + 2], a2);
                if (l0 + q + 3 < k) a3 = fma(gsh[l0 + q + 3], tv[q + 3], a3);
            }
        }
        const double acc = (a0 + a1) + (a2 + a3);
        const double numer = (red[j] - acc) - p.reg_t_l1;
        if (mode == 0) x = fmax(numer, 0.0) / (c + p.eps);
        else if (mode == 1) x = (-numer + c < 0.0) ? p.t_row_sum : 0.0;
        else { x = numer; mx = numer; }
        xraw[j] = x;
        if (mode == 1 || (mode == 0 && !project)) T[(i64)t * ldt + j] = x;
    }
    if (mode != 2) {
        const double s = block_sum(x, scratch);
        if (tid == 0) tpart[blockIdx.x] = s;
    } else {
        i64 idx = (j < d) ? j : (i64)0x7fffffffffffffffLL;
        wave_argmax(mx, idx);
        __shared__ double wm[2];
        __shared__ i64 wi[2];
        if ((tid & 63) == 0) { wm[tid >> 6] = mx; wi[tid >> 6] = idx; }
        __syncthreads();
        if (tid == 0) {
            if (wm[1] > wm[0] || (wm[1] == wm[0] && wi[1] < wi[0])) { wm[0] = wm[1]; wi[0] = wi[1]; }
            tpart[blockIdx.x] = wm[0];
            tpart_idx[blockIdx.x] = wi[0];
        }
    }
    if (blockIdx.x == 0 && tid == 0) st->tmode = mode;
}

__global__ __launch_bounds__(1024) void k_trow_early(double* __restrict__ T, i64 ldt, int d, int k, int t,
                                                     const double* __restrict__ red, i64 ldz,
                                                     const double* __restrict__ wfp, int ntiles, int twfin,
                                                     double* __restrict__ xraw, double* __restrict__ tpart,
                                                     double* __restrict__ Tearly, int check_prev, int tprev,
                                                     int sweep, KParams p, DevState* st) {
    static_assert(TROW_EARLY_COLS == 256, "16 waves: 4 topic residues x 4 column waves");
    if (st->halt) return;
    const int tid = threadIdx.x, lane = tid & 63, wave = tid >> 6, q = wave & 3, cw = wave >> 2;
    __shared__ double scratch[40];
    __shared__ double gsh[RRI_MAX_K];
    __shared__ double ash[4][256];
    __shared__ double xsh[256];
    __shared__ double wsum[4];
    __shared__ double psh[4][RRI_MAX_K];
    static_assert(RRI_MAX_K <= 1024, "a thread per topic");
    const int cl = cw * 64 + lane;
    const i64 j = (i64)blockIdx.x * 256 + cl;
    const bool in = j < d;
    constexpr int CH = 16;
    double tv0[CH];
#pragma unroll
    for (int i = 0; i < CH; ++i) tv0[i] = (q + 4 * i < k && in) ? T[(i64)(q + 4 * i) * ldt + j] : 0.0;
    const double zj = (q == 0 && in) ? red[j] : 0.0;
    const double gl = tid < k ? red_gram(red, ldz, k, tid) : 0.0;
    const double nw = red_gram(red, ldz, k, k);
    double gprev = 0.0, colsum = 0.0;
    if (wfp) {
        const double ga = ordered_sum<2>(wfp, 1, tid, ntiles, 1024);
        const double gb = ordered_sum<2>(wfp + ntiles, 1, tid, ntiles, 1024);
        const double wa = wave_sum<double>(ga), wb = wave_sum<double>(gb);
        if (lane == 0) { scratch[wave] = wa; scratch[16 + wave] = wb; }
        __syncthreads();
        for (int i = 0; i < 16; ++i) { gprev += scratch[i]; colsum += scratch[16 + i]; }
        colsum += red_gram(red, ldz, k, k + 1);
    } else if (check_prev) colsum = red_gram(red, ldz, k, k + 1);
    if (check_prev) {
        const int code = wcol_code(colsum, p);
        if (code != 0) {
            if (blockIdx.x == 0 && tid == 0) halt_set(st, code, tprev, sweep, t);
            return;
        }
    }
    const double c = nw + p.reg_t_l2;
    const int mode = trow_denominator_mode(c, p);
    if (mode < 0) {
        if (blockIdx.x == 0 && tid == 0) halt_set(st, mode, t, sweep, t);
        return;
    }
    if (tid < k) gsh[tid] = (tid == t) ? 0.0 : ((wfp && tid == twfin) ? gprev + gl : gl);
    __syncthreads();
    double a = 0.0;
#pragma unroll
    for (int i = 0; i < CH; ++i)
        if (q + 4 * i < k) a = fma(gsh[q + 4 * i], tv0[i], a);
    for (int l0 = q + 4 * CH; l0 < k; l0 += 4 * CH) {
        double tv[CH];
#pragma unroll
        for (int i = 0; i < CH; ++i) tv[i] = (l0 + 4 * i < k && in) ? T[(i64)(l0 + 4 * i) * ldt + j] : 0.0;
#pragma unroll
        for (int i = 0; i < CH; ++i)
            if (l0 + 4 * i < k) a = fma(gsh[l0 + 4 * i], tv[i], a);
    }
    ash[q][cl] = a;
    __syncthreads();
    if (q == 0) {
        double x = 0.0;
        if (in) {
            const double acc = (ash[0][cl] + ash[1][cl]) + (ash[2][cl] + ash[3][cl]);
            const double numer = (zj - acc) - p.reg_t_l1;
            if (mode == 0) x = fmax(numer, 0.0) / (c + p.eps);
            else x = (-numer + c < 0.0) ? p.t_row_sum : 0.0;
            xraw[j] = x;
            T[(i64)t * ldt + j] = x;
        }
        xsh[cl] = x;
        const double ws = wave_sum<double>(x);
        if (lane == 0) wsum[cw] = ws;
    }
    __syncthreads();
    const double x = xsh[cl];
    if (tid < 2 && ((i64)blockIdx.x * 2 + tid) * 128 < d) tpart[blockIdx.x * 2 + tid] = (0.0 + wsum[2 * tid]) + wsum[2 * tid + 1];
#pragma unroll
    for (int i = 0; i < CH; ++i) {
        const int l = q + 4 * i;
        if (l < k) {
            const double s = wave_sum<double>((l == t ? x : tv0[i]) * x);
            if (lane == 0) psh[cw][l] = s;
        }
    }
    for (int l0 = q + 4 * CH; l0 < k; l0 += 4 * CH) {
        double tv[CH];
#pragma unroll
        for (int i = 0; i < CH; ++i) {
            const int l = l0 + 4 * i;
            tv[i] = (l < k && in && l != t) ? T[(i64)l * ldt + j] : 0.0;
        }
#pragma unroll
        for (int i = 0; i < CH; ++i) {
            const int l = l0 + 4 * i;
            if (l < k) {
                const double s = wave_sum<double>((l == t ? x : tv[i]) * x);
                if (lane == 0) psh[cw][l] = s;
            }
        }
    }
    __syncthreads();
    for (int l = tid; l < k; l += 1024) Tearly[(i64)blockIdx.x * k + l] = (psh[0][l] + psh[1][l]) + (psh[2][l] + psh[3][l]);
    if (blockIdx.x == 0 && tid == 0) st->tmode = mode;
}

__global__ __launch_bounds__(1024) void k_trow_small(double* __restrict__ T, i64 ldt, int d, int k, int t,
                                                     const double* __restrict__ Zpart, int nrb,
                                                     const double* __restrict__ Gpart, int nwb, double* __restrict__ red,
                                                     i64 ldz, double* __restrict__ xraw, double* __restrict__ tpart,
                                                     i64* __restrict__ tpart_idx, int check_prev, int tprev, int sweep,
                                                     KParams p, DevState* st, int resid_form, double* __restrict__ told) {
    if (st->halt) return;
    const int tid = threadIdx.x;
    __shared__ double sh[32 * 33];
    __shared__ double gsh[RRI_MAX_K + 2];
    __shared__ double zs[32];
    const int cc = tid & 31, g = tid >> 5;
    const i64 j = (i64)blockIdx.x * 32 + cc;
    constexpr int ZB = 16;
    double zpre[ZB];
#pragma unroll
    for (int q = 0; q < ZB; ++q) {
        const int r = g + 32 * q;
        zpre[q] = (j < ldz && r < nrb) ? Zpart[(i64)r * ldz + j] : 0.0;
    }
    double tkeep[4];
#pragma unroll
    for (int q = 0; q < 4; ++q) {
        const int l = g + 32 * q;
        tkeep[q] = (j < d && l < k && (l != t || resid_form)) ? T[(i64)l * ldt + j] : 0.0;
    }
    for (int l0 = 0; l0 < k + 2; l0 += 32) {
        const int l = l0 + cc;
        double a = 0.0;
        if (l < k + 2) a = ordered_sum<8>(Gpart + l, k + 2, g, nwb, 32);
        __syncthreads();
        sh[g * 33 + cc] = a;
        __syncthreads();
        if (tid < 32 && l < k + 2) {
            double s = 0.0;
            for (int q = 0; q < 32; ++q) s += sh[q * 33 + tid];
            gsh[l] = s;
        }
    }
    __syncthreads();
    const double nw = gsh[k];
    if (check_prev) {
        const int code = wcol_code(gsh[k + 1], p);
        if (code != 0) {
            if (blockIdx.x == 0 && tid == 0) halt_set(st, code, tprev, sweep, t);
            return;
        }
    }
    const double c = nw + p.reg_t_l2;
    const bool project = p.project_T && p.has_trs;
    const int mode = trow_denominator_mode(c, p);
    if (mode < 0) {
        if (blockIdx.x == 0 && tid == 0) halt_set(st, mode, t, sweep, t);
        return;
    }
    if (blockIdx.x == 0)
        for (int i = tid; i < GRAM_SLICES * (k + 2); i += 1024) red[ldz + i] = i < k + 2 ? gsh[i] : 0.0;
    {
        double a = 0.0;
#pragma unroll
        for (int q = 0; q < ZB; ++q) a += zpre[q];
        if (j < ldz) a = ordered_sum_acc<8>(a, Zpart + j, ldz, g + 32 * ZB, nrb, 32);
        sh[g * 33 + cc] = a;
    }
    __syncthreads();
    if (tid < 32) {
        double s = 0.0;
        for (int q = 0; q < 32; ++q) s += sh[q * 33 + tid];
        zs[tid] = s;
        if (j < ldz) red[j] = s;
    }
    __syncthreads();
    {
        double a = 0.0;
        if (j < d)
            for (int l0 = g; l0 < k; l0 += 32 * 4) {
                double tv[4];
#pragma unroll
                for (int q = 0; q < 4; ++q) {
                    const int l = l0 + 32 * q;
// ... 894 lines not shown
```

### rri_nmf_amd/csrc/rri_layout.hpp

```cpp
#pragma once
#include <algorithm>
#include <cstdint>
#include <string>
#include <vector>

#include "rri_hip.h"

namespace rri {

typedef long long i64;
inline i64 round_up(i64 a, i64 b) { return (a + b - 1) / b * b; }

constexpr size_t dtype_size(int dt) { return dt == RRI_F32 ? 4 : dt == RRI_F64 ? 8 : dt == RRI_F16 ? 2 : dt == RRI_U8 ? 1 : 0; }
constexpr int load_elems(int dt) { return dt == RRI_U8 ? 8 : dtype_size(dt) ? (int)(16 / dtype_size(dt)) : 0; }
constexpr int load_bytes(int dt) { return load_elems(dt) * (int)dtype_size(dt); }

constexpr int WCOL_TILES = 1;
constexpr int GRAM_SLICES = RRI_GRAM_SLICES;
constexpr int TG_ROWS = 32;
constexpr int SP_BLOCK_BYTES = 120 * 1024;
constexpr i64 spx_block_cap() { return (i64)(SP_BLOCK_BYTES / 8 - 64) / 64 * 64; }
struct SpWork { int blk, s0, s1, pad; };
constexpr int ONCHIP_THREADS = 512, ONCHIP_WAVES = ONCHIP_THREADS / 64;
constexpr int ONCHIP_SMALL_K = 22;
constexpr int ONCHIP_MAX_K = 64;
constexpr int ONCHIP_CWA = 32;
constexpr int ONCHIP_PG = ONCHIP_THREADS / ONCHIP_CWA;

constexpr double PASS_CACHE_MB = 256.0;
constexpr int PK_ROWS_MAX = 512;

struct rri_switches {
    bool onchip = true;
    bool onchip_obj = true;
    bool wsweep = true;
    bool trow_fused = true;
    bool obj_direct = false;
    bool wmcorr_cols = true;
    bool wnw_mask = true;
    int pass_rot = -1;
    int rot_cal = 1;
    bool rot_debug = false;
    bool mask_bits = true;
    double pass_cache_mb = PASS_CACHE_MB;
    int pk_rows = 0;
    int pk_il = -1;
    int x_pack = -1;
    bool early_sums = true;
};

struct SpDims { int nblk = 1, bw = 1; i64 nseg = 0, gdim = 0; };
inline SpDims sp_dims(i64 n, i64 d, int which, bool sparse_x, size_t es) {
    const i64 block_bytes = SP_BLOCK_BYTES;
    const i64 cap = sparse_x ? std::min<i64>(spx_block_cap(), std::max<i64>(64, (block_bytes / 8 - 64) / 64 * 64))
                             : block_bytes / (3 * (i64)es);
    SpDims s;
    s.gdim = which == 0 ? d : n;
    s.nseg = which == 0 ? n : d;
    s.nblk = (int)((s.gdim + cap - 1) / cap);
    s.bw = (int)round_up((s.gdim + s.nblk - 1) / s.nblk, 64);
    return s;
}
inline int sp_target_items(int n_cu, bool sparse_x) { return std::max(1, sparse_x ? n_cu / 2 : n_cu); }

inline bool ro_pass_interleaved(int ro_il, int npanels, int nrb) { return ro_il >= 0 ? ro_il != 0 : npanels * nrb <= 1024; }
inline bool wtrow_small(bool has_comm, int nrb) { return !has_comm && nrb <= 64; }

struct DensePlan {
    i64 n = 0, d = 0, LD = 0;
    int k = 0, dtype = RRI_F32, weighted = 0;
    bool explicit_resid = false, sparse_x = false, sparse = false;
    int VN = 4, PW = 1024, kp = 8;
    int npanels = 1, rpb = 1, nrb = 1, nwb = 1, nwb256 = 1, ntb = 1, ntb32 = 1, nsplit = 4;
    i64 red_elems = 0;
    int ro_il = -1;
    int cpart_rows = 0;
    i64 gpart_rows = 1, ttpart_rows = 1, tpart_rows = 1;
    int xy_stride = 1;
    SpDims sp[2];
    int nte = 1, e_blocks = 1, e_tpb = 1, nwfin = 1;
};

constexpr int TROW_EARLY_COLS = 256;
constexpr int WFIN_TILES = 16;
inline int early_job_blocks(i64 n, int n_cu) { return (int)std::max<i64>(1, std::min<i64>((n + 63) / 64, std::max(n_cu, 4) / 4)); }
inline int early_job_first(int pass_blocks, int n_cu) { return std::min(pass_blocks, 4 * std::max(n_cu, 1)); }
inline size_t early_job_lds_doubles(int k) { return (size_t)(2 * k + 2 + 256); }

inline DensePlan dense_plan(i64 n, i64 d, int k, int dtype, int flavour, const rri_switches& sw, int n_cu) {
    DensePlan p;
    p.explicit_resid = flavour == RRI_UNWEIGHTED_RESIDUAL;
    p.sparse_x = flavour == RRI_UNWEIGHTED_SPARSE;
    const int weighted = (p.explicit_resid || p.sparse_x) ? (int)RRI_UNWEIGHTED : flavour;
    const bool explicit_resid = p.explicit_resid;
    p.n = n; p.d = d; p.k = k; p.dtype = dtype; p.weighted = weighted;
    p.sparse = weighted == RRI_WEIGHTED_SPARSE || p.sparse_x;
    p.kp = (int)round_up(k, 8);
    p.VN = load_elems(dtype);
    p.PW = 64 * p.VN * 4;
    p.LD = round_up(d, p.VN);

    p.npanels = (int)((p.LD + p.PW - 1) / p.PW);
    const i64 rpb_cap = ((40 * 1024 - 4 * 8 * 72 * 8) / ((weighted ? 11 : explicit_resid ? 7 : 5) * 8)) / 16 * 16;
    i64 rpb = 0;
    {
        const bool rmw = explicit_resid || weighted == RRI_WEIGHTED_DENSE;
        const int total_max = weighted == RRI_WEIGHTED_DENSE ? 16384 : rmw ? 8192 : 1024;
        const i64 rows_min = weighted == RRI_WEIGHTED_DENSE ? 48 : rmw ? 96 : 192;
        for (int total = total_max; total >= 512 && rpb == 0; total -= 512) {
            const int nrb_t = std::max(1, total / p.npanels);
            const i64 r = (n + nrb_t - 1) / nrb_t;
            if (r >= rows_min || total == 512) rpb = r;
        }
    }
    rpb = std::max<i64>(rpb, 32);
    rpb = std::min<i64>(round_up(rpb, 16), rpb_cap);
    if (dtype == RRI_F32 && !weighted && !explicit_resid && !p.sparse) {
        rpb = sw.pk_rows > 0 ? std::min<i64>(round_up(std::max(sw.pk_rows, 16), 16), rpb_cap) : std::min<i64>(rpb, PK_ROWS_MAX);
        if (sw.pk_rows > 0) p.ro_il = sw.pk_il;
    }
    p.rpb = (int)rpb;
    p.nrb = (int)((n + rpb - 1) / rpb);
    if (p.sparse) {
        for (int w = 0; w < 2; ++w) p.sp[w] = sp_dims(n, d, w, p.sparse_x, dtype_size(dtype));
        p.npanels = p.sp[0].nblk;
        p.nrb = p.sp[1].nblk;
    }
    p.nwb = (int)((n + 64 * WCOL_TILES - 1) / (64 * WCOL_TILES));
    p.nwb256 = (int)((n + 255) / 256);
    p.ntb = (int)((d + 127) / 128);
    p.ntb32 = (int)((p.LD + 31) / 32);
// ... 239 lines not shown
```

### rri_nmf_amd/csrc/rri_onchip_kernels.hpp

```cpp
#pragma once
#include "rri_kernels.hpp"
#include "rri_layout.hpp"

namespace rri {

enum { HALT_ERR_GRID_SYNC = -8 };

struct OnchipArgs {
    const void* X; i64 ldx; int n, d, LD, k;
    double* Wt; i64 ldw; double* T; i64 ldt;
    double* mkZ;
    double* mkG;
    double* mkP;
    double* mkT;
    double* mkX;
    double* xyp; int xy_stride;
    double* objE;
    int track;
    double* objhist;
    double* dec;
    double obj_prev, stop_scale, half_xsq;
    unsigned* bar;
    int G, NA, rows_wg, CG, RG, kS;
    int s0, t0, ph0, s_end;
    int skip_row_finish;
    unsigned spin_limit;
    int nap_eighths;
    unsigned entry_spin_limit;
    unsigned jitter;
    int fail_step;
    long long* dbg;
    KParams p; DevState* st;
};

#define RRI_AGENT __HIP_MEMORY_SCOPE_AGENT
__device__ __forceinline__ void st_agent(double* p, double v) {
    __hip_atomic_store(reinterpret_cast<unsigned long long*>(p), (unsigned long long)__double_as_longlong(v), __ATOMIC_RELAXED, RRI_AGENT);
}
__device__ __forceinline__ double ld_agent(const double* p) {
    return __longlong_as_double((long long)__hip_atomic_load(reinterpret_cast<const unsigned long long*>(p), __ATOMIC_RELAXED, RRI_AGENT));
}

constexpr unsigned ONCHIP_ABSENT_HI = 0xfff7a5a5u, ONCHIP_HALTED_HI = 0xfff7a5a6u;
__device__ __forceinline__ bool onchip_absent(double v) { return (unsigned)__double2hiint(v) == ONCHIP_ABSENT_HI; }
__device__ __forceinline__ bool onchip_halted(double v) { return (unsigned)__double2hiint(v) == ONCHIP_HALTED_HI; }
__device__ __forceinline__ double onchip_absent_value() { return __hiloint2double((int)ONCHIP_ABSENT_HI, (int)ONCHIP_ABSENT_HI); }
__device__ __forceinline__ double onchip_halted_value() { return __hiloint2double((int)ONCHIP_HALTED_HI, (int)ONCHIP_HALTED_HI); }
__device__ __forceinline__ void st_data(double* p, double v) {
    const unsigned hi = (unsigned)__double2hiint(v);
    st_agent(p, (hi == ONCHIP_ABSENT_HI || hi == ONCHIP_HALTED_HI) ? __longlong_as_double(0x7ff8000000000000LL) : v);
}
__device__ __forceinline__ void onchip_stores_landed() { asm volatile("s_waitcnt vmcnt(0)" ::: "memory"); }
__device__ __forceinline__ void onchip_jitter(unsigned seed, int b, int wave, unsigned step, unsigned site) {
    if (seed == 0u) return;
    unsigned h = seed ^ ((unsigned)b * 0x9E3779B1u) ^ ((unsigned)wave * 0x85EBCA77u) ^ (step * 0xC2B2AE3Du) ^ (site * 0x27D4EB2Fu);
    h ^= h >> 15; h *= 0x2C1B3C6Du; h ^= h >> 12; h *= 0x297A2D39u; h ^= h >> 15;
    const int naps = (int)(h % 10u);
    for (int i = 0; i < naps; ++i) __builtin_amdgcn_s_sleep(20);
}

constexpr unsigned ONCHIP_NONE = 0xffffffffu;
struct OnchipNap {
    int ticks = 0;
    long long t0 = 0;
    __device__ __forceinline__ void before() {
        t0 = wall_clock64();
        const long long until = t0 + ticks;
        while (wall_clock64() < until) __builtin_amdgcn_s_sleep(4);
    }
    __device__ __forceinline__ void after(int rounds, int eighths) {
        const int waited = (int)min(wall_clock64() - t0, 0x3fffffffLL);
        ticks = rounds > 0 ? (min(waited, 3276) * eighths) >> 3 : (ticks * 3) >> 2;
    }
};
template <int N, typename OffFn>
__device__ __forceinline__ void onchip_poll_issue(const double* base, OffFn off, double (&v)[N]) {
    int z;
    asm volatile("v_mov_b32 %0, 0" : "=v"(z));
#pragma unroll
    for (int u = 0; u < N; ++u) {
        const unsigned o = off(u, z);
        v[u] = o != ONCHIP_NONE ? ld_agent(base + o) : 0.0;
    }
}
template <int N, typename OffFn>
__device__ __forceinline__ int onchip_poll_finish(const double* base, OffFn off, double (&v)[N], unsigned* bar, unsigned spin_limit,
                                                  int* rounds = nullptr) {
    unsigned spins = 0;
    for (;;) {
        bool ok = true;
#pragma unroll
        for (int u = 0; u < N; ++u) ok = ok && !onchip_absent(v[u]);
        if (__all(ok)) {
            if (rounds) *rounds = (int)spins;
            return 0;
        }
        if ((++spins & 15u) == 0u && __hip_atomic_load(bar, __ATOMIC_RELAXED, RRI_AGENT) != 0u) return 2;
        if (spins > spin_limit) {
            if ((threadIdx.x & 63) == 0) __hip_atomic_store(bar, 1u, __ATOMIC_RELAXED, RRI_AGENT);
            return 2;
        }
        __builtin_amdgcn_s_sleep(2);
        onchip_poll_issue<N>(base, off, v);
    }
}

__device__ __forceinline__ void onchip_signal(unsigned* mine, unsigned value) {
    asm volatile("s_waitcnt vmcnt(0)" ::: "memory");
    __syncthreads();
    if (threadIdx.x == 0) __hip_atomic_store(mine, value, __ATOMIC_RELAXED, RRI_AGENT);
}
__device__ __forceinline__ int onchip_wait(unsigned* bar, const unsigned* flags, int count, unsigned epoch, unsigned spin_limit) {
    __shared__ int verdict_sh;
    if (threadIdx.x < 64) {
        int verdict = 0;
        unsigned spins = 0;
        for (;;) {
            bool ok = true;
            unsigned top = 0u;
            for (int q = threadIdx.x; q < count; q += 64) {
                const unsigned f = __hip_atomic_load(flags + q, __ATOMIC_RELAXED, RRI_AGENT);
                ok = ok && ((f & 0x7fffffffu) >= epoch);
                top |= f & 0x80000000u;
            }
            if (__all(ok)) { verdict = __any(top != 0u) ? 1 : 0; break; }
            if (__hip_atomic_load(bar, __ATOMIC_RELAXED, RRI_AGENT) != 0u) { verdict = 2; break; }
            if (++spins > spin_limit) {
                if (threadIdx.x == 0) __hip_atomic_store(bar, 1u, __ATOMIC_RELAXED, RRI_AGENT);
                verdict = 2;
                break;
            }
            __builtin_amdgcn_s_sleep(1);
        }
        if (threadIdx.x == 0) verdict_sh = verdict;
// ... 674 lines not shown
```

### rri_nmf_amd/engine.py

```python
import collections
import ctypes as C
import re

import numpy as np

from . import _capi
from ._capi import Params, Event

EPS_DIV = float(np.spacing(10))

_NP2RRI = {np.dtype(np.float32): _capi.RRI_F32, np.dtype(np.float64): _capi.RRI_F64, np.dtype(np.float16): _capi.RRI_F16,
           np.dtype(np.uint8): _capi.RRI_U8}
_READ_ONLY = (np.dtype(np.float16), np.dtype(np.uint8))
_HOST_TYPES = (np.dtype(np.float32), np.dtype(np.float64))
_RESET_CODES = {None: _capi.RESET_NONE, 'max_resid_document': _capi.RESET_MAX_RESID_DOCUMENT,
                'random': _capi.RESET_RANDOM}


RankResult = collections.namedtuple('RankResult', 'indptr indices rank val eligible')


class ZeroTotalRows(ValueError):

    def __init__(self, count):
# ... 1139 lines not shown
                for i in at:
                    r[i] = 0.0
                r[at[0]] = max(nw, 0.0)
            if draw is not None:
                self.reduce_write(r)
            self.topic_finish(t)
            if self._stepping_event() is not None:
                self.topic_finish_w(t)
        self.topic_reduce_local(0)
        self.topic_finish(-1)
        self._stepping_event()

    def _row_stride(self):
        vn = 8 if self.dtype == np.uint8 else 16 // self.dtype.itemsize
        return -(-self.d // vn) * vn

    def _topic_sums(self, t, ld, with_wR=True):
        d, k = self.d, self.k
        if self.weighted:
            r = self.reduce_read(2 * ld)
            trow = self.get_T()[t, :]
            nw = r[ld:ld + d]
            return r, r[:d] + trow * nw, nw, trow
        r = self.reduce_read(ld + _capi.RRI_GRAM_SLICES * (k + 2))
        nw = float(sum(r[ld + g * (k + 2) + k] for g in range(_capi.RRI_GRAM_SLICES)))
        wR = None
        if with_wR:
            wW = sum(r[ld + g * (k + 2):ld + g * (k + 2) + k] for g in range(_capi.RRI_GRAM_SLICES))
            wW[t] = 0.0
            wR = r[:d] - wW.dot(self.get_T())
        return r, wR, nw, None

    def topic_sums(self, t):
        ld = self._row_stride()
        self.topic_reduce_local(t)
        _, wR, nw, _ = self._topic_sums(t, ld)
        return np.array(wR), (np.array(nw) if self.weighted else nw)

    def topic_finish_w(self, t):
        self._check(self._lib.rri_topic_finish_w(self._h, int(t)))

    def poll(self):
        return self._check(self._lib.rri_poll(self._h))

    def pending_event(self):
        ev = Event()
        self._check(self._lib.rri_pending_event(self._h, C.byref(ev)))
        return ev.kind, ev.topic, ev.resume_topic

    def resid_row_argmax(self):
        val, row = C.c_double(0.0), C.c_int64(-1)
        self._check(self._lib.rri_resid_row_argmax(self._h, C.byref(val), C.byref(row)))
        return float(val.value), int(row.value)

    def reset_row(self, local_row):
        out = np.empty(self.d, dtype=np.float64)
        self._check(self._lib.rri_reset_row(self._h, int(local_row), out.ctypes.data_as(C.POINTER(C.c_double))))
        return out

    def apply_reset_vectors(self, t, T_row, W_col):
        T_row = np.ascontiguousarray(T_row, dtype=np.float64)
        W_col = np.ascontiguousarray(W_col, dtype=np.float64)
        self._check(self._lib.rri_apply_reset_vectors(
            self._h, int(t), T_row.ctypes.data_as(C.POINTER(C.c_double)),
            W_col.ctypes.data_as(C.POINTER(C.c_double))))
        self.n_resets_used += 1

    def timing_enable(self, on=True, every=1):
        self._check(self._lib.rri_timing_enable(self._h, int(every) if on else 0))

    def timing_read(self, kernel_id):
        cnt, ms = C.c_int64(0), C.c_double(0.0)
        self._check(self._lib.rri_timing_read(self._h, int(kernel_id), C.byref(cnt), C.byref(ms)))
        return int(cnt.value), float(ms.value)

    def onchip_info(self):
        el, n = C.c_int32(0), C.c_int64(0)
        self._check(self._lib.rri_onchip_info(self._h, C.byref(el), C.byref(n)))
        return bool(el.value), int(n.value)

    LAYOUT_COPY_FIELDS = ('nblk', 'bw', 'lps', 'nwork')
    LAYOUT_FIELDS = ('rpb', 'nrb', 'npanels', 'mask_bits', 'mask_cols', 'mask_density', 'wtrow_small', 'nw_from_mask',
                     'interleaved', 'wcorr_nrb', 'n_cu', 'x_pack', 'x_pack_base', 'x_pack_flagged', 'x_pack_tiles', 'x_pack_bits',
                     'x_pack_book', 'x_pack_exceptions', 'early_sums', 'early_steps')
    assert 2 * len(LAYOUT_COPY_FIELDS) + len(LAYOUT_FIELDS) == _capi.RRI_LAYOUT_FIELDS

    def layout_info(self):
        nc = len(self.LAYOUT_COPY_FIELDS)
        out = (C.c_int64 * _capi.RRI_LAYOUT_FIELDS)()
        self._check(self._lib.rri_layout_info(self._h, out, _capi.RRI_LAYOUT_FIELDS))
        v = [int(x) for x in out]
        info = {name: (v[i], v[nc + i]) for i, name in enumerate(self.LAYOUT_COPY_FIELDS)}
        info.update(zip(self.LAYOUT_FIELDS, v[2 * nc:]))
        for name in ('mask_bits', 'mask_cols', 'wtrow_small', 'nw_from_mask', 'interleaved', 'x_pack', 'early_sums'):
            info[name] = bool(info[name])
        info['mask_density'] = None if info['mask_density'] < 0 else info['mask_density'] * 1e-9
        info['x_pack_book'] = [info['x_pack_book'] >> (8 * i) & 0xff for i in range(7)] if info['x_pack_bits'] == 26 else []
        return info

    def debug_xcc(self, count=32):
        out = (C.c_int32 * count)()
        self._check(self._lib.rri_debug_xcc(self._h, out, count))
        return list(out)

    def onchip_fallbacks(self):
        n = C.c_int64(0)
        self._check(self._lib.rri_onchip_fallbacks(self._h, C.byref(n)))
        return int(n.value)

    def sweep_until(self, n_sweeps, obj_prev, stop_scale):
        n_sweeps = int(n_sweeps)
        if not self.onchip_info()[0]:
            return None
        hist = np.full(n_sweeps, np.nan, dtype=np.float64)
        done = C.c_int32(0)
        st = self._lib.rri_sweep_until(self._h, n_sweeps, float(obj_prev), float(stop_scale),
                                       hist.ctypes.data_as(C.POINTER(C.c_double)), C.byref(done))
        if st == _capi.RRI_ERR_UNSUPPORTED:
            return None
        n_done = self._drive(st, done)
        return n_done, hist[:n_done]

    def synchronize(self):
        self._check(self._lib.rri_synchronize(self._h))

    def bench_rank1_update(self, reps=5):
        ms = C.c_double(0.0)
        self._check(self._lib.rri_bench_rank1_update(self._h, int(reps), C.byref(ms)))
        return float(ms.value)

    def bench_stream_copy(self, reps=5):
        ms = C.c_double(0.0)
        self._check(self._lib.rri_bench_stream_copy(self._h, int(reps), C.byref(ms)))
        return float(ms.value)
```

Before: 36.45.

## Compute early T-gram partials inside the pass kernel with polled on-chip handoff

Moves the per-block T·T[t,:] partial sums out of k_trow_early and into extra blocks of the fused pass kernel. The early-sum blocks poll a double-buffered Tearly array with agent-scope loads, using sentinel values to detect missing data. A bounded poll count drops to a slow path in k_wfin, which recomputes the Gram entries and dot products directly and counts how often this happens. The intent is to shorten the trow_early critical path and overlap that work with the pass. In exchange it adds spin-waiting, relies on co-residency between blocks of one launch, and changes launch bounds for the EJ variant.

```diff
diff --git a/include/rri_hip.h b/include/rri_hip.h
--- a/include/rri_hip.h
+++ b/include/rri_hip.h
@@ -189,7 +189,7 @@
 rri_status rri_timing_read(rri_ctx* ctx, int32_t kernel_id, int64_t* launches, double* total_ms);
 rri_status rri_synchronize(rri_ctx* ctx);
 rri_status rri_onchip_info(rri_ctx* ctx, int32_t* eligible, int64_t* launches);
-#define RRI_LAYOUT_FIELDS 28
+#define RRI_LAYOUT_FIELDS 29
 rri_status rri_layout_info(rri_ctx* ctx, int64_t* out, int32_t n);
 rri_status rri_onchip_fallbacks(rri_ctx* ctx, int64_t* fallbacks);
 rri_status rri_device_memory(int64_t* buffers, int64_t* bytes);
diff --git a/rri_nmf_amd/_capi.py b/rri_nmf_amd/_capi.py
--- a/rri_nmf_amd/_capi.py
+++ b/rri_nmf_amd/_capi.py
@@ -5,7 +5,7 @@
 LIB_PATH = os.environ.get('RRI_HIP_LIB', os.path.join(_PKG, 'lib', 'librri_hip.so'))
 
 RRI_GRAM_SLICES = 8
-RRI_LAYOUT_FIELDS = 28
+RRI_LAYOUT_FIELDS = 29
 RRI_MAX_K = 1024
 RRI_MAX_TOPN = 64
 RRI_MAX_COOC_WORDS = 32
diff --git a/rri_nmf_amd/csrc/rri_hip.hip b/rri_nmf_amd/csrc/rri_hip.hip
--- a/rri_nmf_amd/csrc/rri_hip.hip
+++ b/rri_nmf_amd/csrc/rri_hip.hip
@@ -231,6 +231,8 @@
     bool carry_valid = false;
     int carry_topic = -1;
     double *Tearly = nullptr, *edot = nullptr, *Gearly = nullptr, *ent = nullptr, *wfp = nullptr;
+    unsigned* einfo = nullptr;
+    int early_buf = 0;
     bool early_valid = false, carry_wfin = false;
     int early_topic = -1, wfin_topic = -1;
     long early_steps = 0;
@@ -1040,16 +1042,27 @@
                early_job_lds_doubles(c->k) <= 5 * (size_t)c->rpb + 4 * 8 * 72;
     }
     static EarlyJob early_job(const rri_ctx* c, int t, int tn) {
-        return EarlyJob{(const double*)c->W, c->ldw, (int)c->n, c->k, t, tn, (const double*)c->Tearly, c->plan.nte, c->edot,
-                        c->Gearly, c->ent, early_job_first(c->npanels * c->nrb, c->n_cu), c->plan.e_blocks, c->plan.e_tpb};
+        return EarlyJob{(const double*)c->W, c->ldw, (int)c->n, c->k, t, tn, (const double*)tearly_buf(c, c->early_buf), c->plan.nte, c->edot,
+                        c->Gearly, c->ent, early_job_first(c->npanels * c->nrb, c->n_cu), c->plan.e_blocks, c->plan.e_tpb,
+                        c->einfo + 2, c->sw.early_poll_rounds >= 0 ? c->sw.early_poll_rounds : EARLY_POLL_ROUNDS};
+    }
+    static double* tearly_buf(const rri_ctx* c, int which) { return c->Tearly + (size_t)which * c->plan.nte * c->k; }
+    static TgramJob early_tgram(const rri_ctx* c, TgramJob job) {
+        job.Tearly = tearly_buf(c, c->early_buf);
+        job.nte = c->plan.nte;
+        job.nblocks += job.nte;
+        return job;
     }
     static void wfin(rri_ctx* c, int t, int tn, int sweep) {
         TimedScope ts(c, 1);
         const int nredb = (int)((c->LD + 31) / 32) + GRAM_SLICES;
         hipLaunchKernelGGL(k_wfin, dim3(nredb + c->plan.nwfin), dim3(1024), 0, c->stream, c->W, c->ldw, (int)c->n, c->k, t, tn,
                            (const double*)c->Ypart, c->npanels, (const double*)c->edot, (const double*)c->ent, c->Gpart,
-                           c->wfp, c->nwb, c->XYpart + (i64)t * c->xy_stride, (const double*)c->Zpart, c->LD, c->nrb, (const double*)c->Gearly,
-                           c->plan.e_blocks, c->red, nredb, sweep, kparams(c), c->st);
+                           c->wfp, c->nwb, c->XYpart + (i64)t * c->xy_stride, (const double*)c->Zpart, c->LD, c->nrb, c->Gearly,
+                           c->plan.e_blocks, c->red, nredb, sweep, kparams(c), c->st, (const unsigned*)(c->einfo + 2),
+                           (const double*)tearly_buf(c, c->early_buf), c->plan.nte, c->plan.e_tpb, tearly_buf(c, c->early_buf ^ 1), c->ent,
+                           reinterpret_cast<unsigned long long*>(c->einfo));
+        c->early_buf ^= 1;
         c->gpart_n = c->nwb;
         c->early_steps += 1;
         note_xy(c, t, c->nwb * WCOL_TILES);
@@ -1057,7 +1070,7 @@
     static void trow_early(rri_ctx* c, int t, int check_prev, int tprev, int sweep) {
         hipLaunchKernelGGL(k_trow_early, dim3(c->plan.nte), dim3(1024), 0, c->stream, c->T, c->LD, (int)c->d, c->k, t,
                            (const double*)c->red, c->LD, c->carry_wfin ? (const double*)c->wfp : (const double*)nullptr, c->nwb,
-                           c->wfin_topic, c->xraw, c->tpart, c->Tearly, check_prev, tprev, sweep, kparams(c), c->st);
+                           c->wfin_topic, c->xraw, c->tpart, check_prev, tprev, sweep, kparams(c), c->st);
         c->tpart_n = c->ntb;
     }
     static void trow(rri_ctx* c, int t, int check_prev, int tprev, int sweep, bool force_final) {
@@ -1440,7 +1453,7 @@
     }
     const bool early = carry_next && LK::early_ok(c) && c->early_valid && c->early_topic == t;
     if (carry_next) {
-        DISPATCH_RO(c, (L::template pass<true, true>(c, t, tn, job, early ? LK::early_job(c, t, tn) : EarlyJob{})));
+        DISPATCH_RO(c, (L::template pass<true, true>(c, t, tn, early ? LK::early_tgram(c, job) : job, early ? LK::early_job(c, t, tn) : EarlyJob{})));
         if (early) LK::wfin(c, t, tn, sweep);
         else LK::wcol<true, true>(c, t, tn, sweep);
         c->carry_valid = true;
@@ -2159,6 +2172,7 @@
     if (const char* e = getenv("RRI_PASS_CACHE_MB")) sw.pass_cache_mb = std::max(0.0, atof(e));
     if (const char* e = getenv("RRI_X_PACK")) sw.x_pack = atoi(e) == 2 ? 2 : atoi(e) != 0;
     if (const char* e = getenv("RRI_EARLY_SUMS")) sw.early_sums = atoi(e) != 0;
+    if (const char* e = getenv("RRI_EARLY_POLL_ROUNDS")) sw.early_poll_rounds = std::max(0, atoi(e));
     if (const char* e = getenv("RRI_PASS_PK_GEOM")) {
         char* end = nullptr;
         sw.pk_rows = (int)std::min<long>(std::max<long>(0, strtol(e, &end, 10)), 1 << 20);
@@ -2308,10 +2322,12 @@
     CR(dev_alloc(c, c->dtmp, 16 * f8));
     CR(dev_alloc(c, c->itmp, 16 * sizeof(i64)));
     if (c->sw.early_sums && !weighted && !explicit_resid && !p.sparse && k > 1) {
-        CR(dev_alloc(c, c->Tearly, (size_t)p.nte * k * f8, true));
+        CR(dev_alloc(c, c->Tearly, (size_t)2 * p.nte * k * f8));
+        CR(hipMemsetD32Async((hipDeviceptr_t)c->Tearly, (int)ONCHIP_ABSENT_HI, (size_t)2 * p.nte * k * 2, c->stream));
         CR(dev_alloc(c, c->edot, (size_t)n * f8, true));
         CR(dev_alloc(c, c->Gearly, (size_t)p.e_blocks * (k + 2) * f8, true));
-        CR(dev_alloc(c, c->ent, 8 * f8, true));
+        CR(dev_alloc(c, c->ent, (size_t)(8 + (2 + p.e_blocks + 1) / 2) * f8, true));
+        c->einfo = reinterpret_cast<unsigned*>(c->ent + 8);
         CR(dev_alloc(c, c->wfp, (size_t)2 * c->nwb * f8, true));
     }
     const bool keeps_resid = explicit_resid || (weighted && !c->sparse);
@@ -5368,6 +5384,11 @@
     CHECK_CTX(c);
     if (!out || n < 1) return fail(c, RRI_ERR_INVALID, "rri_layout_info needs room for at least one value");
     const bool dense_w = c->weighted == RRI_WEIGHTED_DENSE;
+    unsigned long long early_slow = 0;
+    if (c->einfo) {
+        HIPCHK(c, hipStreamSynchronize(c->stream));
+        HIPCHK(c, hipMemcpy(&early_slow, c->einfo, sizeof(early_slow), hipMemcpyDeviceToHost));
+    }
     const int64_t v[RRI_LAYOUT_FIELDS] = {
         c->sparse ? c->sp[0].nblk : 0, c->sparse ? c->sp[0].bw : 0, c->sparse ? c->sp[0].lps : 0, c->sparse ? c->sp[0].nwork : 0,
         c->sparse ? c->sp[1].nblk : 0, c->sparse ? c->sp[1].bw : 0, c->sparse ? c->sp[1].lps : 0, c->sparse ? c->sp[1].nwork : 0,
@@ -5381,7 +5402,7 @@
         c->xp_valid ? 1 : 0, c->xp_valid ? c->xp_base : 0, c->xp_flagged, c->xp_tiles,
         c->xp_valid ? (c->xn_valid ? 26 : 28) : 0, c->xn_valid ? (int64_t)((uint64_t)c->xn_books.hi << 32 | c->xn_books.lo) : 0,
         c->xn_exceptions,
-        LK::early_ok(c) ? 1 : 0, c->early_steps};
+        LK::early_ok(c) ? 1 : 0, c->early_steps, (int64_t)early_slow};
     for (int i = 0; i < n && i < RRI_LAYOUT_FIELDS; ++i) out[i] = v[i];
     return RRI_OK;
 }
diff --git a/rri_nmf_amd/csrc/rri_kernels.hpp b/rri_nmf_amd/csrc/rri_kernels.hpp
--- a/rri_nmf_amd/csrc/rri_kernels.hpp
+++ b/rri_nmf_amd/csrc/rri_kernels.hpp
@@ -94,11 +94,30 @@
     else *p = v;
 }
 
+#define RRI_AGENT __HIP_MEMORY_SCOPE_AGENT
+__device__ __forceinline__ void st_agent(double* p, double v) {
+    __hip_atomic_store(reinterpret_cast<unsigned long long*>(p), (unsigned long long)__double_as_longlong(v), __ATOMIC_RELAXED, RRI_AGENT);
+}
+__device__ __forceinline__ double ld_agent(const double* p) {
+    return __longlong_as_double((long long)__hip_atomic_load(reinterpret_cast<const unsigned long long*>(p), __ATOMIC_RELAXED, RRI_AGENT));
+}
+
+constexpr unsigned ONCHIP_ABSENT_HI = 0xfff7a5a5u, ONCHIP_HALTED_HI = 0xfff7a5a6u;
+__device__ __forceinline__ bool onchip_absent(double v) { return (unsigned)__double2hiint(v) == ONCHIP_ABSENT_HI; }
+__device__ __forceinline__ bool onchip_halted(double v) { return (unsigned)__double2hiint(v) == ONCHIP_HALTED_HI; }
+__device__ __forceinline__ double onchip_absent_value() { return __hiloint2double((int)ONCHIP_ABSENT_HI, (int)ONCHIP_ABSENT_HI); }
+__device__ __forceinline__ double onchip_halted_value() { return __hiloint2double((int)ONCHIP_HALTED_HI, (int)ONCHIP_HALTED_HI); }
+__device__ __forceinline__ void st_data(double* p, double v) {
+    const unsigned hi = (unsigned)__double2hiint(v);
+    st_agent(p, (hi == ONCHIP_ABSENT_HI || hi == ONCHIP_HALTED_HI) ? __longlong_as_double(0x7ff8000000000000LL) : v);
+}
+
 struct TgramJob {
     const double* T; i64 ldt; int d, k, t;
     double* Ttpart; const double* tpart; int ntb, nsplit, finish, sweep;
     KParams p; DevState* st;
     int nblocks;
+    double* Tearly = nullptr; int nte = 0;
 };
 __device__ __forceinline__ void tgram_block(const double* __restrict__ T, i64 ldt, int d, int k, int t, int l, int split,
                                             int ns, double* __restrict__ Ttpart, const double* __restrict__ tpart,
@@ -123,12 +142,42 @@
     }
 }
 
+__device__ __forceinline__ void tearly_block(const double* __restrict__ T, i64 ldt, int d, int k, int t, int b,
+                                             double* __restrict__ Tearly, double* psh) {
+    const int tid = threadIdx.x, lane = tid & 63, cw = tid >> 6;
+    const i64 j = (i64)b * TROW_EARLY_COLS + tid;
+    const bool in = j < d;
+    const double x = in ? T[(i64)t * ldt + j] : 0.0;
+    constexpr int CH = 8, LC = 64;
+    for (int lc = 0; lc < k; lc += LC) {
+        const int l1 = min(k, lc + LC);
+        for (int l0 = lc; l0 < l1; l0 += CH) {
+            double tv[CH];
+#pragma unroll
+            for (int i = 0; i < CH; ++i) tv[i] = (l0 + i < l1 && in && l0 + i != t) ? T[(i64)(l0 + i) * ldt + j] : 0.0;
+#pragma unroll
+            for (int i = 0; i < CH; ++i) {
+                const int l = l0 + i;
+                if (l < l1) {
+                    const double s = wave_sum<double>((l == t ? x : tv[i]) * x);
+                    if (lane == 0) psh[cw * LC + l - lc] = s;
+                }
+            }
+        }
+        __syncthreads();
+        if (tid < l1 - lc) st_data(Tearly + (i64)b * k + lc + tid, (psh[tid] + psh[LC + tid]) + (psh[2 * LC + tid] + psh[3 * LC + tid]));
+        __syncthreads();
+    }
+}
+
 struct EarlyJob {
     const double* Wt; i64 ldw; int n, k, t, tn;
     const double* Tearly; int nte;
     double *dot, *Gpart, *nt;
     int first, nblocks, tpb;
+    unsigned* inval; int poll_rounds;
 };
+constexpr int EARLY_POLL_ROUNDS = 1 << 14;
 template <int CH>
 __device__ __forceinline__ void early_block(const EarlyJob& e, int b, double* sm) {
     const int tid = threadIdx.x, lane = tid & 63, wave = tid >> 6, k = e.k, t = e.t;
@@ -136,8 +185,28 @@
     double* gsh = tts + k;
     double* dsh = gsh + k + 2;
     for (int l = tid; l < k + 2; l += 256) gsh[l] = 0.0;
-    for (int l = tid; l < k; l += 256) tts[l] = ordered_sum<8>(e.Tearly + l, k, 0, e.nte, 1);
-    __syncthreads();
+    bool there = true;
+    for (int l = tid; l < k && there; l += 256) {
+        for (int round = 0;; ++round) {
+            if (round >= e.poll_rounds) { there = false; break; }
+            if (round > 0) __builtin_amdgcn_s_sleep(16);
+            bool ok = true;
+            double a = 0.0;
+            for (int i = 0; i < e.nte; i += 8) {
+                double v[8];
+#pragma unroll
+                for (int q = 0; q < 8; ++q) v[q] = i + q < e.nte ? ld_agent(e.Tearly + (i64)(i + q) * k + l) : 0.0;
+#pragma unroll
+                for (int q = 0; q < 8; ++q) { ok = ok && !onchip_absent(v[q]); a += v[q]; }
+            }
+            if (ok) { tts[l] = a; break; }
+        }
+    }
+    if (__syncthreads_or(there ? 0 : 1)) {
+        if (tid == 0) __hip_atomic_store(e.inval + b, 1u, __ATOMIC_RELAXED, RRI_AGENT);
+        return;
+    }
+    if (tid == 0) __hip_atomic_store(e.inval + b, 0u, __ATOMIC_RELAXED, RRI_AGENT);
     if (b == 0 && tid == 0) e.nt[0] = tts[t];
     __syncthreads();
     if (tid == 0) tts[t] = 0.0;
@@ -333,7 +402,7 @@
     }
 
 template <typename SX, bool DO_Y, bool DO_Z, int UPD, int U, bool NT, bool RS, int PK = 0, bool EJ = false>
-__global__ __launch_bounds__(256) void k_pass(typename std::conditional<(UPD > 0), SX, const SX>::type* __restrict__ X,
+__global__ __launch_bounds__(256, (EJ && sizeof(SX) == 4) ? 4 : 1) void k_pass(typename std::conditional<(UPD > 0), SX, const SX>::type* __restrict__ X,
                                               i64 ldx, int n, int ncols,
                                               const double* __restrict__ trow, const double* __restrict__ wcol,
                                               double* __restrict__ Ypart, double* __restrict__ Zpart, i64 ldz,
@@ -359,6 +428,14 @@
     if (st->halt) return;
     if ((int)blockIdx.x < job.nblocks) {
         __shared__ double jscratch[40];
+        if constexpr (EJ) {
+            if ((int)blockIdx.x >= job.nblocks - job.nte) {
+                extern __shared__ __attribute__((aligned(16))) unsigned char jsmem[];
+                tearly_block(job.T, job.ldt, job.d, job.k, job.t, (int)blockIdx.x - (job.nblocks - job.nte), job.Tearly,
+                             reinterpret_cast<double*>(jsmem));
+                return;
+            }
+        }
         tgram_block(job.T, job.ldt, job.d, job.k, job.t, (int)blockIdx.x % job.k, (int)blockIdx.x / job.k, job.nsplit,
                     job.Ttpart, job.tpart, job.ntb, job.finish, job.sweep, job.p, job.st, jscratch);
         return;
@@ -1040,21 +1117,64 @@
 
 __global__ __launch_bounds__(1024) void k_wfin(double* __restrict__ Wt, i64 ldw, int n, int k, int t, int tn,
                                                const double* __restrict__ Ypart, int npanels,
-                                               const double* __restrict__ dot, const double* __restrict__ nt,
+                                               const double* __restrict__ dot, const double* nt,
                                                double* __restrict__ Gtile, double* __restrict__ wfp, int ntiles,
                                                double* __restrict__ xyp, const double* __restrict__ Zpart, i64 ldz, int nrb,
-                                               const double* __restrict__ Gearly, int ne, double* __restrict__ red,
-                                               int nredb, int sweep, KParams p, DevState* st) {
+                                               double* Gearly, int ne, double* __restrict__ red,
+                                               int nredb, int sweep, KParams p, DevState* st,
+                                               const unsigned* __restrict__ inval, const double* __restrict__ Tearly, int nte,
+                                               int tpb, double* __restrict__ Tmark, double* ntw,
+                                               unsigned long long* __restrict__ nslow) {
     static_assert(WFIN_TILES == 16 && WCOL_TILES == 1, "a wave per tile, a row of Gtile and an entry of xyp per tile");
+    static_assert(RRI_MAX_K <= 32 * 33, "T T[t,:]^T of the slow path in sh");
+    const int lane = threadIdx.x & 63, wave = threadIdx.x >> 6;
+    if ((int)blockIdx.x >= nredb) {
+        const int nmark = nte * k, nth = ((int)gridDim.x - nredb) * 1024;
+        for (int e = ((int)blockIdx.x - nredb) * 1024 + (int)threadIdx.x; e < nmark; e += nth) Tmark[e] = onchip_absent_value();
+    }
     if (st->halt) return;
     __shared__ double sh[32 * 33];
+    bool gave_up = false;
+    for (int e = lane; e < ne; e += 64) gave_up = gave_up || inval[e] != 0u;
+    const bool slow = __any(gave_up) != 0;
     if ((int)blockIdx.x < nredb) {
+        const int gs = (int)blockIdx.x - (nredb - GRAM_SLICES);
+        if (slow && gs >= 0) {
+            const int per = (ne + GRAM_SLICES - 1) / GRAM_SLICES;
+            const int tiles_all = (n + 63) / 64;
+            for (int r = gs * per; r < min(ne, (gs + 1) * per); ++r) {
+                const int tile1 = min(tiles_all, (r + 1) * tpb);
+                for (int l = wave; l < k + 2; l += 16) {
+                    double acc = 0.0;
+                    if (l != t && l != k + 1) {
+                        for (int tile = r * tpb; tile < tile1; ++tile) {
+                            const i64 i = (i64)tile * 64 + lane;
+                            const double wn = i < n ? Wt[(i64)tn * ldw + i] : 0.0;
+                            const double wl = l == k ? wn : (i < n ? Wt[(i64)l * ldw + i] : 0.0);
+                            acc += wave_sum<double>(wn * wl);
+                        }
+                    }
+                    if (lane == 0) Gearly[(i64)r * (k + 2) + l] = acc;
+                }
+            }
+            __threadfence_block();
+            __syncthreads();
+        }
         reduce_block((int)blockIdx.x, nredb, Zpart, ldz, nrb, Gearly, ne, k, red, sh);
         return;
     }
     const int b = (int)blockIdx.x - nredb;
-    const int lane = threadIdx.x & 63, wave = threadIdx.x >> 6;
-    const double cden = nt[0] + p.reg_w_l2;
+    double nt0;
+    if (slow) {
+        for (int l = threadIdx.x; l < k; l += 1024) sh[l] = ordered_sum<8>(Tearly + l, k, 0, nte, 1);
+        __syncthreads();
+        nt0 = sh[t];
+        __syncthreads();
+        if (threadIdx.x == 0) sh[t] = 0.0;
+        __syncthreads();
+        if (b == 0 && threadIdx.x == 0) { ntw[0] = nt0; nslow[0] += 1ull; }
+    } else nt0 = nt[0];
+    const double cden = nt0 + p.reg_w_l2;
     const int mode = wcol_denominator_mode(cden, p);
     if (mode < 0) {
         if (b == 0 && threadIdx.x == 0) halt_set(st, mode, t, sweep, t);
@@ -1067,7 +1187,18 @@
     double wn = 0.0, y = 0.0, wnew = 0.0;
     if (valid) {
         wn = Wt[(i64)tn * ldw + i];
-        const double dt = dot[i];
+        double dt;
+        if (slow) {
+            double a[4] = {0.0, 0.0, 0.0, 0.0};
+            for (int l0 = 0; l0 < k; l0 += 4) {
+#pragma unroll
+                for (int q = 0; q < 4; ++q) {
+                    const int l = l0 + q;
+                    if (l < k) a[q] = fma(l != t ? Wt[(i64)l * ldw + i] : 0.0, sh[l], a[q]);
+                }
+            }
+            dt = (a[0] + a[1]) + (a[2] + a[3]);
+        } else dt = dot[i];
         y = ordered_sum<8>(Ypart + i, n, 0, npanels, 1);
         const double numer = (y - dt) - p.reg_w_l1;
         if (mode == 0) wnew = fmax(numer, 0.0) / (cden + p.eps);
@@ -1167,17 +1298,14 @@
                                                      const double* __restrict__ red, i64 ldz,
                                                      const double* __restrict__ wfp, int ntiles, int twfin,
                                                      double* __restrict__ xraw, double* __restrict__ tpart,
-                                                     double* __restrict__ Tearly, int check_prev, int tprev,
-                                                     int sweep, KParams p, DevState* st) {
+                                                     int check_prev, int tprev, int sweep, KParams p, DevState* st) {
     static_assert(TROW_EARLY_COLS == 256, "16 waves: 4 topic residues x 4 column waves");
     if (st->halt) return;
     const int tid = threadIdx.x, lane = tid & 63, wave = tid >> 6, q = wave & 3, cw = wave >> 2;
     __shared__ double scratch[40];
     __shared__ double gsh[RRI_MAX_K];
     __shared__ double ash[4][256];
-    __shared__ double xsh[256];
     __shared__ double wsum[4];
-    __shared__ double psh[4][RRI_MAX_K];
     static_assert(RRI_MAX_K <= 1024, "a thread per topic");
     const int cl = cw * 64 + lane;
     const i64 j = (i64)blockIdx.x * 256 + cl;
@@ -1238,39 +1366,11 @@
             xraw[j] = x;
             T[(i64)t * ldt + j] = x;
         }
-        xsh[cl] = x;
         const double ws = wave_sum<double>(x);
         if (lane == 0) wsum[cw] = ws;
     }
     __syncthreads();
-    const double x = xsh[cl];
     if (tid < 2 && ((i64)blockIdx.x * 2 + tid) * 128 < d) tpart[blockIdx.x * 2 + tid] = (0.0 + wsum[2 * tid]) + wsum[2 * tid + 1];
-#pragma unroll
-    for (int i = 0; i < CH; ++i) {
-        const int l = q + 4 * i;
-        if (l < k) {
-            const double s = wave_sum<double>((l == t ? x : tv0[i]) * x);
-            if (lane == 0) psh[cw][l] = s;
-        }
-    }
-    for (int l0 = q + 4 * CH; l0 < k; l0 += 4 * CH) {
-        double tv[CH];
-#pragma unroll
-        for (int i = 0; i < CH; ++i) {
-            const int l = l0 + 4 * i;
-            tv[i] = (l < k && in && l != t) ? T[(i64)l * ldt + j] : 0.0;
-        }
-#pragma unroll
-        for (int i = 0; i < CH; ++i) {
-            const int l = l0 + 4 * i;
-            if (l < k) {
-                const double s = wave_sum<double>((l == t ? x : tv[i]) * x);
-                if (lane == 0) psh[cw][l] = s;
-            }
-        }
-    }
-    __syncthreads();
-    for (int l = tid; l < k; l += 1024) Tearly[(i64)blockIdx.x * k + l] = (psh[0][l] + psh[1][l]) + (psh[2][l] + psh[3][l]);
     if (blockIdx.x == 0 && tid == 0) st->tmode = mode;
 }
 
diff --git a/rri_nmf_amd/csrc/rri_layout.hpp b/rri_nmf_amd/csrc/rri_layout.hpp
--- a/rri_nmf_amd/csrc/rri_layout.hpp
+++ b/rri_nmf_amd/csrc/rri_layout.hpp
@@ -47,6 +47,7 @@
     int pk_il = -1;
     int x_pack = -1;
     bool early_sums = true;
+    int early_poll_rounds = -1;
 };
 
 struct SpDims { int nblk = 1, bw = 1; i64 nseg = 0, gdim = 0; };
diff --git a/rri_nmf_amd/csrc/rri_onchip_kernels.hpp b/rri_nmf_amd/csrc/rri_onchip_kernels.hpp
--- a/rri_nmf_amd/csrc/rri_onchip_kernels.hpp
+++ b/rri_nmf_amd/csrc/rri_onchip_kernels.hpp
@@ -33,23 +33,6 @@
     KParams p; DevState* st;
 };
 
-#define RRI_AGENT __HIP_MEMORY_SCOPE_AGENT
-__device__ __forceinline__ void st_agent(double* p, double v) {
-    __hip_atomic_store(reinterpret_cast<unsigned long long*>(p), (unsigned long long)__double_as_longlong(v), __ATOMIC_RELAXED, RRI_AGENT);
-}
-__device__ __forceinline__ double ld_agent(const double* p) {
-    return __longlong_as_double((long long)__hip_atomic_load(reinterpret_cast<const unsigned long long*>(p), __ATOMIC_RELAXED, RRI_AGENT));
-}
-
-constexpr unsigned ONCHIP_ABSENT_HI = 0xfff7a5a5u, ONCHIP_HALTED_HI = 0xfff7a5a6u;
-__device__ __forceinline__ bool onchip_absent(double v) { return (unsigned)__double2hiint(v) == ONCHIP_ABSENT_HI; }
-__device__ __forceinline__ bool onchip_halted(double v) { return (unsigned)__double2hiint(v) == ONCHIP_HALTED_HI; }
-__device__ __forceinline__ double onchip_absent_value() { return __hiloint2double((int)ONCHIP_ABSENT_HI, (int)ONCHIP_ABSENT_HI); }
-__device__ __forceinline__ double onchip_halted_value() { return __hiloint2double((int)ONCHIP_HALTED_HI, (int)ONCHIP_HALTED_HI); }
-__device__ __forceinline__ void st_data(double* p, double v) {
-    const unsigned hi = (unsigned)__double2hiint(v);
-    st_agent(p, (hi == ONCHIP_ABSENT_HI || hi == ONCHIP_HALTED_HI) ? __longlong_as_double(0x7ff8000000000000LL) : v);
-}
 __device__ __forceinline__ void onchip_stores_landed() { asm volatile("s_waitcnt vmcnt(0)" ::: "memory"); }
 __device__ __forceinline__ void onchip_jitter(unsigned seed, int b, int wave, unsigned step, unsigned site) {
     if (seed == 0u) return;
diff --git a/rri_nmf_amd/engine.py b/rri_nmf_amd/engine.py
--- a/rri_nmf_amd/engine.py
+++ b/rri_nmf_amd/engine.py
@@ -1245,7 +1245,7 @@
     LAYOUT_COPY_FIELDS = ('nblk', 'bw', 'lps', 'nwork')
     LAYOUT_FIELDS = ('rpb', 'nrb', 'npanels', 'mask_bits', 'mask_cols', 'mask_density', 'wtrow_small', 'nw_from_mask',
                      'interleaved', 'wcorr_nrb', 'n_cu', 'x_pack', 'x_pack_base', 'x_pack_flagged', 'x_pack_tiles', 'x_pack_bits',
-                     'x_pack_book', 'x_pack_exceptions', 'early_sums', 'early_steps')
+                     'x_pack_book', 'x_pack_exceptions', 'early_sums', 'early_steps', 'early_slow_steps')
     assert 2 * len(LAYOUT_COPY_FIELDS) + len(LAYOUT_FIELDS) == _capi.RRI_LAYOUT_FIELDS
 
     def layout_info(self):
```

After: 36.78 (median of 6 runs). Within noise of the previous version (+0.9%).
